# FurkanOM/tf-rpn

Hardware: AMD Instinct MI355X
Metric: proposal images/sec at 500x500x3 VOC batch; NMS boxes/sec (higher is better)
Workload: dtype f16x3; 1 GPU; configs[1]: 500x500x3 synthetic batch=8 per GPU, vgg16 backbone + RPN head, 9 anchors/cell, decode + NMS(300), 1xMI355X; per_gpu_batch=8, global_batch=8, img_size=500, anchors_per_image=8649, nms_topn=300, weights=random-init (seeded He-normal), parallelism=image-sharded dp1, one RCCL all-gather of proposals, nms_overlap=decode+NMS of step k on a second HIP stream, overlapping the convs of step k+1

## Files before the change

### tf_rpn_amd/csrc/conv_split_kernels.hip

```cpp
#include "conv_kernels.h"

#include <cmath>
#include <cstdlib>
#include <cstring>
#include <mutex>
#include <unordered_map>

#ifndef RPN_PIN
#define RPN_PIN 1
#endif
#if RPN_PIN
#define RPN_PIN_LOADS() __builtin_amdgcn_sched_barrier(0)
#else
#define RPN_PIN_LOADS() ((void)0)
#endif

#ifdef RPN_STAMP
__device__ unsigned long long g_rpn_stamps[8192 * 32];
#define RPN_STAMP_AT(k)                                                                                    \
    do {                                                                                                   \
        if (threadIdx.x == 0 && blockIdx.x < 8192 && (k) < 32)                                             \
            g_rpn_stamps[blockIdx.x * 32 + (k)] = __builtin_readcyclecounter();                            \
    } while (0)
#define RPN_STAMP_VAL(k, v)                                                                                \
    do {                                                                                                   \
        if (threadIdx.x == 0 && blockIdx.x < 8192) g_rpn_stamps[blockIdx.x * 32 + (k)] = (v);             \
    } while (0)
extern "C" int rpn_debug_read_stamps(unsigned long long *out, int n)
{
    return (int)hipMemcpyFromSymbol(out, HIP_SYMBOL(g_rpn_stamps), (size_t)n * 8);
}
#else
#define RPN_STAMP_AT(k) ((void)0)
#define RPN_STAMP_VAL(k, v) ((void)0)
#endif

namespace rpn {

__device__ __forceinline__ void wave_sync()
{
    __builtin_amdgcn_fence(__ATOMIC_RELEASE, "wavefront");
    __builtin_amdgcn_wave_barrier();
    __builtin_amdgcn_fence(__ATOMIC_ACQUIRE, "wavefront");
}

using f32x16 = __attribute__((ext_vector_type(16))) float;
using bf16x8 = __attribute__((ext_vector_type(8))) __bf16;
using f16x8 = __attribute__((ext_vector_type(8))) _Float16;
using u32x4 = __attribute__((ext_vector_type(4))) unsigned;

constexpr int TWS = 32;
constexpr int HW = TWS + 2;
constexpr int kStagePad = 4;

template <bool F16> struct Half;
template <> struct Half<false> {
    using vec = bf16x8;
    using elem = __bf16;
    static __device__ __forceinline__ f32x16 mfma(u32x4 a, u32x4 b, f32x16 c)
    {
        return __builtin_amdgcn_mfma_f32_32x32x16_bf16(__builtin_bit_cast(bf16x8, a), __builtin_bit_cast(bf16x8, b), c,
                                                       0, 0, 0);
    }
};
template <> struct Half<true> {
    using vec = f16x8;
    using elem = _Float16;
    static __device__ __forceinline__ f32x16 mfma(u32x4 a, u32x4 b, f32x16 c)
    {
        return __builtin_amdgcn_mfma_f32_32x32x16_f16(__builtin_bit_cast(f16x8, a), __builtin_bit_cast(f16x8, b), c, 0,
                                                      0, 0);
    }
};

template <bool F16>
__device__ __forceinline__ uint4 split_piece(const float (&x)[8], bool lo, unsigned *status = nullptr)
{
    using E = typename Half<F16>::elem;
    typename Half<F16>::vec v;
    if constexpr (F16) {
        if (status && !lo) {
            const float m = fmaxf(fmaxf(fmaxf(fabsf(x[0]), fabsf(x[1])), fmaxf(fabsf(x[2]), fabsf(x[3]))),
                                  fmaxf(fmaxf(fabsf(x[4]), fabsf(x[5])), fmaxf(fabsf(x[6]), fabsf(x[7]))));
            float nan_probe = 0.0f;
#pragma unroll
            for (int k = 0; k < 8; ++k) nan_probe = fmaf(x[k], 0.0f, nan_probe);
            if (!(m <= 65504.0f) || nan_probe != 0.0f) atomicOr(status, 1u );
        }
    }
#pragma unroll
    for (int k = 0; k < 8; ++k) {
        const E h = (E)x[k];
        v[k] = lo ? (E)(x[k] - (float)h) : h;
    }
    return __builtin_bit_cast(uint4, v);
}

template <bool F16>
__device__ __forceinline__ float join(unsigned short hi, unsigned short lo)
{
    using E = typename Half<F16>::elem;
    return (float)__builtin_bit_cast(E, hi) + (float)__builtin_bit_cast(E, lo);
}

using f32x4 = __attribute__((ext_vector_type(4))) float;

template <bool F16>
__device__ __forceinline__ f32x4 mfma16(u32x4 a, u32x4 b, f32x4 c)
{
    if constexpr (F16)
        return __builtin_amdgcn_mfma_f32_16x16x32_f16(__builtin_bit_cast(f16x8, a), __builtin_bit_cast(f16x8, b), c, 0, 0, 0);
    else
        return __builtin_amdgcn_mfma_f32_16x16x32_bf16(__builtin_bit_cast(bf16x8, a), __builtin_bit_cast(bf16x8, b), c, 0, 0, 0);
}

__device__ __forceinline__ int halo_swz(int hx) { return hx & 6; }

__device__ __forceinline__ int xcd_remap_s(int bid, int nwg)
{
    const int q = nwg >> 3, r = nwg & 7, xcd = bid & 7;
    return (xcd < r ? xcd * (q + 1) : r * (q + 1) + (xcd - r) * q) + (bid >> 3);
}

struct SplitConvArgs {
    const uint4 *x;
    const uint4 *w;
    const float *bias;
    void *out;
    int B, H, W, Cin, Cout, cout_pad;
    float out_scale;
    int act, out_f32;
    unsigned *sched;
    unsigned *status;
    const float *img;
    const uint4 *w1;
    const float *b1;
    float scale1;
    long long slab_floats;
    int ktree;
};

template <int TH, int WN, int BBUF, int NW, bool F16, bool POOL, bool B1 = false>
__global__ void __launch_bounds__(64 * NW, NW / 2)
conv3x3_split_kernel(SplitConvArgs a, int tiles_x, int tiles_y, int n_tiles)
{
    constexpr int NT = 64 * NW;
    constexpr int WM = NW / WN;
    constexpr int MI = TH / WM;
    constexpr int NI = 2;
    constexpr int BN = WN * NI * 32;
    constexpr int HP = (TH + 2) * HW;
    constexpr int A_PIECES = HP * 4;
    constexpr int A_ROUNDS = (A_PIECES + NT - 1) / NT;
    constexpr int A_RPS = (A_ROUNDS + 2) / 3;
    constexpr int B_PIECES = 3 * BN * 4;
    constexpr int B_ROUNDS = B_PIECES / NT;
    static_assert(MI * WM == TH && B_PIECES % NT == 0, "tile shape");
    constexpr int STAGE_LD = 64 + kStagePad;
    constexpr int ABUF = HP * 4 + 4;
    constexpr int PW = TWS + 4;
    constexpr int PATCH_F = B1 ? (TH + 4) * PW * 3 : 0;
    static_assert(!B1 || (WN == 1 && POOL && BBUF == 2), "B1: the 64 -> 64 pooled instantiations only");
    constexpr int LDS_PIPE = 2 * ABUF + BBUF * B_PIECES;
    constexpr int LDS_STAGE = (NW * 32 * STAGE_LD * 4 + 15) / 16;
    constexpr int LDS_UINT4 = (LDS_PIPE > LDS_STAGE ? LDS_PIPE : LDS_STAGE) + (PATCH_F + 3) / 4;

    __shared__ uint4 lds[LDS_UINT4];
    u32x4 *As = reinterpret_cast<u32x4 *>(lds);
    u32x4 *Bs = reinterpret_cast<u32x4 *>(lds) + 2 * ABUF;

    const int tid = threadIdx.x;
    const int lane = tid & 63;
    const int wave = tid >> 6;
    const int wm = wave / WN, wn = wave % WN;
    const int lm = lane & 31, kh = lane >> 5;

    int nt, mt;
    {
        const int m_tiles = tiles_x * tiles_y * a.B;
        const int XN = n_tiles >= 8 ? 8 : (n_tiles >= 4 ? 4 : (n_tiles >= 2 ? 2 : 1)), XM = 8 / XN;
        const int NTl = (n_tiles + XN - 1) / XN;
        const int xcd = blockIdx.x & 7, slot = blockIdx.x >> 3;
        nt = (slot % NTl) * XN + (xcd % XN);
        mt = (slot / NTl) * XM + (xcd / XN);
        if (nt >= n_tiles || mt >= m_tiles) return;
    }
    const int tx = mt % tiles_x;
    mt /= tiles_x;
    const int ty = mt % tiles_y;
    const int img = mt / tiles_y;
    const int oy0 = ty * TH, ox0 = tx * TWS, n0 = nt * BN;

    const int chunks = a.Cin >> 4;
    const int steps = chunks * 3;
    const size_t in_pix_stride = (size_t)chunks * 4;
    const uint4 *__restrict__ xin = B1 ? nullptr : a.x + (size_t)img * a.H * a.W * in_pix_stride;

    constexpr int A_SLOTS = 3 * A_RPS;
    constexpr unsigned kOob = 0x80000000u;
    const __amdgpu_buffer_rsrc_t xrsrc = __builtin_amdgcn_make_buffer_rsrc(
        const_cast<uint4 *>(xin), (short)0, (int)((size_t)a.H * a.W * in_pix_stride * 16), 0x00020000);
    unsigned a_goff[A_SLOTS];
    int a_loff[A_SLOTS];
#pragma unroll
    for (int R = 0; R < (B1 ? 0 : A_SLOTS); ++R) {
        const int e = R * NT + tid;
        const int pix = e >> 2, pc = e & 3;
        const int hy = pix / HW, hx = pix - hy * HW;
        const int iy = oy0 - 1 + hy, ix = ox0 - 1 + hx;
        const bool piece = e < A_PIECES;
        const bool inimg = piece && iy >= 0 && iy < a.H && ix >= 0 && ix < a.W;
        a_loff[R] = piece ? (pix * 4 + (pc ^ ((hx >> 2) & 3))) : HP * 4;
        a_goff[R] = inimg ? (unsigned)((((size_t)iy * a.W + ix) * in_pix_stride + pc) * 16) : kOob;
    }
    u32x4 b_reg[B_ROUNDS];
    u32x4 a_reg[A_RPS];
#define RPN_LOAD_B(STEP)                                                                               \
    {                                                                                                  \
        const u32x4 *src_ = reinterpret_cast<const u32x4 *>(a.w) + ((size_t)(STEP) * 3 * a.cout_pad + n0) * 4;   \
        _Pragma("unroll") for (int i_ = 0; i_ < B_ROUNDS; ++i_) {                                      \
            const int e_ = tid + i_ * NT;                                                              \
            const int t_ = e_ / (BN * 4), rem_ = e_ - t_ * (BN * 4);                \
            b_reg[i_] = src_[(size_t)t_ * a.cout_pad * 4 + rem_];                                      \
        }                                                                                              \
    }
#define RPN_STORE_B(BUF)                                                                               \
    {                                                                                                  \
        _Pragma("unroll") for (int i_ = 0; i_ < B_ROUNDS; ++i_) {                                      \
            const int e_ = tid + i_ * NT;                                                              \
            const int t_ = e_ / (BN * 4), rem_ = e_ - t_ * (BN * 4);                                   \
            const int n_ = rem_ >> 2, pc_ = rem_ & 3;                                                  \
            Bs[(((BUF) * 3 + t_) * BN + n_) * 4 + (pc_ ^ ((n_ >> 2) & 3))] = b_reg[i_];                \
        }                                                                                              \
    }
#define RPN_LOAD_A(CHUNK, R) \
    __builtin_bit_cast(u32x4, __builtin_amdgcn_raw_buffer_load_b128(xrsrc, a_goff[R], (CHUNK) * 64, 0))

    constexpr int NBLK = (HP + 15) / 16;
    constexpr int QB = B1 ? (NBLK + NW - 1) / NW : 1;
    constexpr int QPS = (QB + 2) / 3;
    float *patchf = reinterpret_cast<float *>(lds + (LDS_PIPE > LDS_STAGE ? LDS_PIPE : LDS_STAGE));
    const int lr = lane & 15, kg = lane >> 4;
    u32x4 phi[QB], plo[QB];
    int pdst[QB];
    float b1_max = 0.0f;
    unsigned pin = 0;
    u32x4 w1hi = {0, 0, 0, 0}, w1lo = {0, 0, 0, 0};
    f32x4 b1v = {0.f, 0.f, 0.f, 0.f};
    (void)patchf; (void)lr; (void)kg; (void)pin; (void)phi; (void)plo; (void)pdst; (void)w1hi; (void)w1lo; (void)b1v;
    (void)b1_max;
#define RPN_B1_LOADW(CHUNK)                                                                            \
    {                                                                                                  \
        const u32x4 *w1_ = reinterpret_cast<const u32x4 *>(a.w1) + ((CHUNK) * 16 + lr) * 8 + kg;       \
        w1hi = w1_[0];                                                                                 \
        w1lo = w1_[4];                                                                                 \
        b1v = *reinterpret_cast<const f32x4 *>(a.b1 + (CHUNK) * 16 + 4 * kg);                          \
    }
#define RPN_B1_BLOCK(Q, BUF)                                                                           \
    {                                                                                                  \
        f32x4 c_ = {0.f, 0.f, 0.f, 0.f};                                                               \
        c_ = mfma16<F16>(w1lo, phi[Q], c_);                                                            \
        c_ = mfma16<F16>(w1hi, plo[Q], c_);                                                            \
        c_ = mfma16<F16>(w1hi, phi[Q], c_);                                                            \
        using E_ = typename Half<F16>::elem;                                                           \
        using h4_ = __attribute__((ext_vector_type(4))) E_;                                            \
        const bool in_ = (pin >> (Q)) & 1u;                                                            \
        h4_ hv_, lv_;                                                                                  \
        _Pragma("unroll") for (int r_ = 0; r_ < 4; ++r_) {                                             \
            float v_ = fmaxf(c_[r_] * a.scale1 + b1v[r_], 0.0f);                                       \
            v_ = in_ ? v_ : 0.0f;                                                                      \
            b1_max = fmaxf(b1_max, v_);                                                                \
            const E_ h_ = (E_)v_;                                                                      \
            hv_[r_] = h_;                                                                              \
            lv_[r_] = (E_)(v_ - (float)h_);                                                            \
        }                                                                                              \
        char *d_ = reinterpret_cast<char *>(As + (BUF) * ABUF);                                        \
        *reinterpret_cast<uint2 *>(d_ + pdst[Q]) = __builtin_bit_cast(uint2, hv_);                     \
        *reinterpret_cast<uint2 *>(d_ + (pdst[Q] ^ 16)) = __builtin_bit_cast(uint2, lv_);              \
    }
    if constexpr (B1) {
        const float *ximg = a.img + (size_t)img * a.H * a.W * 3;
        for (int e = tid; e < PATCH_F; e += NT) {
            const int pr = e / (PW * 3), rem = e - pr * (PW * 3);
            const int iy = oy0 - 2 + pr, ix = ox0 - 2 + rem / 3;
            patchf[e] = (iy >= 0 && iy < a.H && ix >= 0 && ix < a.W) ? ximg[((size_t)iy * a.W + ix) * 3 + rem % 3] : 0.0f;
        }
    }

    f32x16 acc[MI][NI];
#pragma unroll
    for (int i = 0; i < MI; ++i)
#pragma unroll
        for (int j = 0; j < NI; ++j)
#pragma unroll
            for (int e = 0; e < 16; ++e) acc[i][j][e] = 0.0f;

    int a_off[3];
#pragma unroll
    for (int s3 = 0; s3 < 3; ++s3) a_off[s3] = (lm + s3) * 4 + ((2 * kh) ^ (((lm + s3) >> 2) & 3));
    int b_off[NI];
#pragma unroll
    for (int j = 0; j < NI; ++j) {
        const int n = wn * (NI * 32) + j * 32 + lm;
        b_off[j] = n * 4 + ((2 * kh) ^ ((n >> 2) & 3));
    }

    if constexpr (B1) {
        RPN_LOAD_B(0);
        RPN_B1_LOADW(0);
        RPN_STORE_B(0);
        __syncthreads();
        int koff[8];
#pragma unroll
        for (int j = 0; j < 8; ++j) {
            const int k = 8 * kg + j;
            koff[j] = k < 27 ? (k / 9) * (PW * 3) + (k % 9) : -1;
        }
#pragma unroll
        for (int q = 0; q < QB; ++q) {
            const int p = (wave + NW * q) * 16 + lr;
            const bool valid = p < HP;
            const int pp = valid ? p : HP - 1;
            const int hy = pp / HW, hx = pp - hy * HW;
            const int base = (hy * PW + hx) * 3;
            float xs[8];
#pragma unroll
            for (int j = 0; j < 8; ++j) xs[j] = koff[j] >= 0 ? patchf[base + koff[j]] : 0.0f;
            phi[q] = __builtin_bit_cast(u32x4, split_piece<F16>(xs, false));
            plo[q] = __builtin_bit_cast(u32x4, split_piece<F16>(xs, true));
            const int iy = oy0 - 1 + hy, ix = ox0 - 1 + hx;
            if (iy >= 0 && iy < a.H && ix >= 0 && ix < a.W) pin |= 1u << q;
            pdst[q] = valid ? (pp * 4 + ((2 * (kg >> 1)) ^ ((hx >> 2) & 3))) * 16 + (kg & 1) * 8 : HP * 4 * 16 + (kg & 1) * 8;
        }
#pragma unroll
        for (int q = 0; q < QB; ++q) RPN_B1_BLOCK(q, 0);
    } else {
#pragma unroll
        for (int R = 0; R < A_SLOTS; ++R) As[a_loff[R]] = RPN_LOAD_A(0, R);
        RPN_LOAD_B(0);
        RPN_STORE_B(0);
    }
    __syncthreads();

    int abuf = 0, bbuf = 0;
#pragma unroll 1
    for (int chunk = 0; chunk < chunks; ++chunk) {
        const int next_chunk = chunk + 1 < chunks ? chunk + 1 : chunk;
#pragma unroll
        for (int row = 0; row < 3; ++row) {
            const int step = chunk * 3 + row;
            RPN_LOAD_B(step + 1 < steps ? step + 1 : step);
            if constexpr (B1) {
                if (row == 0) RPN_B1_LOADW(next_chunk);
            } else {
#pragma unroll
                for (int q = 0; q < A_RPS; ++q) a_reg[q] = RPN_LOAD_A(next_chunk, row * A_RPS + q);
            }
            if constexpr (NW == 4) RPN_PIN_LOADS();

            const u32x4 *arow = As + (abuf * ABUF + (wm * MI + row) * HW * 4);
#pragma unroll
            for (int s = 0; s < 3; ++s) {
                u32x4 ahi[MI], alo[MI], bhi[NI], blo[NI];
#pragma unroll
                for (int i = 0; i < MI; ++i) {
                    ahi[i] = arow[i * HW * 4 + a_off[s]];
                    alo[i] = arow[i * HW * 4 + (a_off[s] ^ 1)];
                }
#pragma unroll
                for (int j = 0; j < NI; ++j) {
                    bhi[j] = Bs[(bbuf * 3 + s) * BN * 4 + b_off[j]];
                    blo[j] = Bs[(bbuf * 3 + s) * BN * 4 + (b_off[j] ^ 1)];
                }
#pragma unroll
                for (int i = 0; i < MI; ++i)
#pragma unroll
                    for (int j = 0; j < NI; ++j) {
                        acc[i][j] = Half<F16>::mfma(alo[i], bhi[j], acc[i][j]);
                        acc[i][j] = Half<F16>::mfma(ahi[i], blo[j], acc[i][j]);
                        acc[i][j] = Half<F16>::mfma(ahi[i], bhi[j], acc[i][j]);
                    }
            }

            if (BBUF == 1) __syncthreads();
            RPN_STORE_B(BBUF == 2 ? (bbuf ^ 1) : 0);
            if constexpr (B1) {
#pragma unroll
                for (int q = row * QPS; q < (row + 1) * QPS && q < QB; ++q) RPN_B1_BLOCK(q, abuf ^ 1);
            } else {
#pragma unroll
                for (int q = 0; q < A_RPS; ++q) As[(abuf ^ 1) * ABUF + a_loff[row * A_RPS + q]] = a_reg[q];
            }
            __syncthreads();
            if (BBUF == 2) bbuf ^= 1;
        }
        abuf ^= 1;
    }

#undef RPN_LOAD_B
#undef RPN_STORE_B
#undef RPN_LOAD_A
#undef RPN_B1_LOADW
#undef RPN_B1_BLOCK
    if constexpr (B1 && F16) {
        if (a.status && !(b1_max <= 65504.0f)) atomicOr(a.status, 1u );
    }
    float *stage = reinterpret_cast<float *>(lds) + wave * (32 * STAGE_LD);
    float bias_v[NI];
#pragma unroll
    for (int j = 0; j < NI; ++j) {
        const int n = n0 + wn * (NI * 32) + j * 32 + lm;
        bias_v[j] = (a.bias && n < a.Cout) ? a.bias[n] : 0.0f;
    }
    const float act_lo = a.act == ACT_LINEAR ? -INFINITY : 0.0f;
    const float act_hi = a.act == ACT_RELU6 ? 6.0f : INFINITY;
    const int cout_chunks = a.Cout >> 4;
    const int nbase = n0 + wn * (NI * 32);
    const int pix_bytes = a.out_f32 ? a.Cout * 4 : cout_chunks * 64;
    auto store_stage = [&](int npx_log2, int oy, int oxb, int OHo, int OWo) {
        if (oy >= OHo) return;
        const long long row_off = (((long long)img * OHo + oy) * OWo + oxb) * (long long)pix_bytes;
        const __amdgpu_buffer_rsrc_t ors = __builtin_amdgcn_make_buffer_rsrc(reinterpret_cast<char *>(a.out) + row_off, (short)0,
                                                                              (OWo - oxb) * pix_bytes, 0x00020000);
        if (a.out_f32) {
            const int rounds = (16 << npx_log2) >> 6;
            const int px_l = lane >> 4, q_l = lane & 15;
            const int n = nbase + 4 * q_l;
            unsigned voff = n < a.Cout ? (unsigned)(px_l * pix_bytes + n * 4) : 0x80000000u;
#pragma unroll
            for (int rd = 0; rd < rounds; ++rd) {
                const u32x4 v = *reinterpret_cast<const u32x4 *>(&stage[(rd * 4 + px_l) * STAGE_LD + 4 * q_l]);
                __builtin_amdgcn_raw_buffer_store_b128(v, ors, voff, 0, 0);
                voff += (unsigned)(4 * pix_bytes);
            }
        } else {
            const int rounds2 = (8 << npx_log2) >> 6;
            const int px2 = lane >> 3, q2 = lane & 7;
            const int cl = q2 >> 1, hf = q2 & 1;
            const int n = nbase + cl * 16;
            unsigned voff = n < a.Cout ? (unsigned)(px2 * pix_bytes + (n >> 4) * 64 + hf * 32) : 0x80000000u;
#pragma unroll
            for (int rd = 0; rd < rounds2; ++rd) {
                float xs[8];
                const float *src = &stage[(rd * 8 + px2) * STAGE_LD + cl * 16 + hf * 8];
                const float4 v0 = *reinterpret_cast<const float4 *>(src);
                const float4 v1 = *reinterpret_cast<const float4 *>(src + 4);
                xs[0] = v0.x; xs[1] = v0.y; xs[2] = v0.z; xs[3] = v0.w;
                xs[4] = v1.x; xs[5] = v1.y; xs[6] = v1.z; xs[7] = v1.w;
                const u32x4 hi = __builtin_bit_cast(u32x4, split_piece<F16>(xs, false, a.status));
                const u32x4 lo = __builtin_bit_cast(u32x4, split_piece<F16>(xs, true, nullptr));
                __builtin_amdgcn_raw_buffer_store_b128(hi, ors, voff, 0, 0);
                __builtin_amdgcn_raw_buffer_store_b128(lo, ors, voff + 16u, 0, 0);
                voff += (unsigned)(8 * pix_bytes);
            }
        }
    };

    if constexpr (POOL) {
        static_assert(!POOL || (MI % 2 == 0), "pooling needs an even number of rows per wave");
        const int OHo = a.H >> 1, OWo = a.W >> 1;
#pragma unroll
        for (int ip = 0; ip < MI / 2; ++ip) {
#pragma unroll
            for (int j = 0; j < NI; ++j)
#pragma unroll
                for (int e2 = 0; e2 < 8; ++e2) {
                    const float v0 = fmaxf(acc[2 * ip][j][2 * e2], acc[2 * ip][j][2 * e2 + 1]);
                    const float v1 = fmaxf(acc[2 * ip + 1][j][2 * e2], acc[2 * ip + 1][j][2 * e2 + 1]);
                    const int m2 = (e2 & 1) + 4 * (e2 >> 1) + 2 * kh;
                    stage[m2 * STAGE_LD + j * 32 + lm] = fminf(fmaxf(fmaxf(v0, v1) * a.out_scale + bias_v[j], act_lo), act_hi);
                }
            wave_sync();
            store_stage(4, (oy0 + wm * MI + 2 * ip) >> 1, ox0 >> 1, OHo, OWo);
            wave_sync();
        }
    } else {
#pragma unroll
        for (int i = 0; i < MI; ++i) {
#pragma unroll
            for (int j = 0; j < NI; ++j)
#pragma unroll
                for (int e = 0; e < 16; ++e) {
                    const int m = (e & 3) + 8 * (e >> 2) + 4 * kh;
                    stage[m * STAGE_LD + j * 32 + lm] = fminf(fmaxf(acc[i][j][e] * a.out_scale + bias_v[j], act_lo), act_hi);
                }
            wave_sync();
            store_stage(5, oy0 + wm * MI + i, ox0, a.H, a.W);
            wave_sync();
        }
    }
}


#ifdef RPN_NOSTORE
#define RPN_STORE_INDEX(i) ((i) & 63)
#else
#define RPN_STORE_INDEX(i) (i)
#endif

template <bool F16, bool POOL, int RW, int NW, int NJ = 4>
__device__ __forceinline__ void split16_epilogue(f32x4 (&acc)[RW * 2][NJ], float *lds_f, const SplitConvArgs &a, int img,
                                                 int oy0, int ox0, int n0, int wave, int wm, int wn, int lane,
                                                 int stamp_base = -1 )
{
    (void)stamp_base;
    asm volatile("" : "+v"(lane));
    constexpr int MT = RW * 2;
    constexpr int CW = 16 * NJ;
    constexpr int STAGE_LD = CW + kStagePad;
    constexpr int PP = CW / 4;
    const int lr = lane & 15, kg = lane >> 4;
    float *stage = lds_f + wave * (32 * STAGE_LD);
    float bias_v[NJ];
#pragma unroll
    for (int j = 0; j < NJ; ++j) {
        const int n = n0 + wn * CW + j * 16 + lr;
        bias_v[j] = (a.bias && n < a.Cout) ? a.bias[n] : 0.0f;
    }
    const float act_lo = a.act == ACT_LINEAR ? -INFINITY : 0.0f;
    const float act_hi = a.act == ACT_RELU6 ? 6.0f : INFINITY;
    const int cout_chunks = a.Cout >> 4;
    const int nbase = n0 + wn * CW;
    const int pix_bytes = a.out_f32 ? a.Cout * 4 : cout_chunks * 64;
    constexpr int PXR = 64 / PP;
    const int px_l = lane / PP, q_l = lane % PP;
    auto store_stage = [&](int npx_log2, int oy, int oxb, int OHo, int OWo) {
        if (oy >= OHo) return;
        const int rounds = (PP << npx_log2) >> 6;
        const long long row_off = (((long long)img * OHo + oy) * OWo + oxb) * (long long)pix_bytes;
        const __amdgpu_buffer_rsrc_t ors = __builtin_amdgcn_make_buffer_rsrc(reinterpret_cast<char *>(a.out) + row_off, (short)0,
                                                                              (OWo - oxb) * pix_bytes, 0x00020000);
        if (a.out_f32) {
            const int n = nbase + 4 * q_l;
            unsigned voff = n < a.Cout ? (unsigned)(px_l * pix_bytes + n * 4) : 0x80000000u;
#pragma unroll
            for (int rd = 0; rd < rounds; ++rd) {
                const u32x4 v = *reinterpret_cast<const u32x4 *>(&stage[(rd * PXR + px_l) * STAGE_LD + 4 * q_l]);
#ifdef RPN_NOSTORE
                __builtin_amdgcn_raw_buffer_store_b128(v, ors, (unsigned)(lane * 16), 0, 0);
#else
                __builtin_amdgcn_raw_buffer_store_b128(v, ors, voff, 0, 0);
#endif
                voff += (unsigned)(PXR * pix_bytes);
            }
        } else {
            constexpr int LPP = CW / 8;
            constexpr int PXR2 = 64 / LPP;
            const int px2 = lane / LPP, q2 = lane % LPP;
            const int cl = q2 >> 1, hf = q2 & 1;
            const int n = nbase + cl * 16;
            unsigned voff = n < a.Cout ? (unsigned)(px2 * pix_bytes + (n >> 4) * 64 + hf * 32) : 0x80000000u;
            const int rounds2 = (1 << npx_log2) / PXR2;
#pragma unroll
            for (int rd = 0; rd < rounds2; ++rd) {
                float xs[8];
                const float *src = &stage[(rd * PXR2 + px2) * STAGE_LD + cl * 16 + hf * 8];
                const float4 v0 = *reinterpret_cast<const float4 *>(src);
                const float4 v1 = *reinterpret_cast<const float4 *>(src + 4);
                xs[0] = v0.x; xs[1] = v0.y; xs[2] = v0.z; xs[3] = v0.w;
                xs[4] = v1.x; xs[5] = v1.y; xs[6] = v1.z; xs[7] = v1.w;
                const u32x4 hi = __builtin_bit_cast(u32x4, split_piece<F16>(xs, false, a.status));
                const u32x4 lo = __builtin_bit_cast(u32x4, split_piece<F16>(xs, true, nullptr));
#ifdef RPN_NOSTORE
                __builtin_amdgcn_raw_buffer_store_b128(hi, ors, (unsigned)(lane * 32), 0, 0);
                __builtin_amdgcn_raw_buffer_store_b128(lo, ors, (unsigned)(lane * 32 + 16), 0, 0);
#else
                __builtin_amdgcn_raw_buffer_store_b128(hi, ors, voff, 0, 0);
                __builtin_amdgcn_raw_buffer_store_b128(lo, ors, voff + 16u, 0, 0);
#endif
                voff += (unsigned)(PXR2 * pix_bytes);
            }
        }
    };

    if constexpr (POOL) {
        const int OHo = a.H >> 1, OWo = a.W >> 1;
#pragma unroll
        for (int hf = 0; hf < 2; ++hf)
#pragma unroll
            for (int j = 0; j < NJ; ++j)
#pragma unroll
                for (int r2 = 0; r2 < 2; ++r2) {
                    const float v0 = fmaxf(acc[hf][j][2 * r2], acc[hf][j][2 * r2 + 1]);
                    const float v1 = fmaxf(acc[(MT - 2) + hf][j][2 * r2], acc[(MT - 2) + hf][j][2 * r2 + 1]);
                    const int px2 = 8 * hf + 2 * kg + r2;
                    stage[px2 * STAGE_LD + j * 16 + lr] = fminf(fmaxf(fmaxf(v0, v1) * a.out_scale + bias_v[j], act_lo), act_hi);
                }
        wave_sync();
        store_stage(4, (oy0 + 2 * wm) >> 1, ox0 >> 1, OHo, OWo);
    } else {
#pragma unroll
        for (int i = 0; i < RW; ++i) {
#pragma unroll
            for (int hf = 0; hf < 2; ++hf)
#pragma unroll
                for (int j = 0; j < NJ; ++j)
#pragma unroll
                    for (int r = 0; r < 4; ++r) {
                        const int px = 16 * hf + 4 * kg + r;
                        stage[px * STAGE_LD + j * 16 + lr] =
                            fminf(fmaxf(acc[i * 2 + hf][j][r] * a.out_scale + bias_v[j], act_lo), act_hi);
                    }
            wave_sync();
            if (stamp_base >= 0) RPN_STAMP_AT(stamp_base + 2 * i);
            store_stage(5, oy0 + RW * wm + i, ox0, a.H, a.W);
            wave_sync();
            if (stamp_base >= 0) RPN_STAMP_AT(stamp_base + 2 * i + 1);
        }
    }
}

template <int TH, int WN, int NW, bool F16, bool POOL>
__global__ void __launch_bounds__(64 * NW, NW == 8 ? 2 : 2)
conv3x3_split16_kernel(SplitConvArgs a, int tiles_x, int tiles_y, int n_tiles)
{
    constexpr int NT = 64 * NW, BN = 64 * WN;
    constexpr int WM = NW / WN, RW = TH / WM;
    constexpr int MT = RW * 2;
    constexpr int HP = (TH + 2) * HW;
    constexpr int PPP = 8;
    constexpr int ABUF = HP * PPP + 8;
    constexpr int A_PIECES = HP * PPP;
    constexpr int A_ROUNDS = (A_PIECES + NT - 1) / NT;
    constexpr int A_RPS = (A_ROUNDS + 2) / 3, A_SLOTS = 3 * A_RPS;
    constexpr int B_PIECES = 3 * BN * PPP;
    constexpr int B_ROUNDS = B_PIECES / NT;
    constexpr int STAGE_LD = 64 + kStagePad;
    constexpr int LDS_PIPE = 2 * ABUF + B_PIECES;
    constexpr int LDS_STAGE = (NW * 32 * STAGE_LD * 4 + 15) / 16;
    constexpr int LDS_UINT4 = LDS_PIPE > LDS_STAGE ? LDS_PIPE : LDS_STAGE;
    static_assert(RW * WM == TH && RW >= 1 && B_PIECES % NT == 0 && (!POOL || RW == 2), "tile shape");

    __shared__ uint4 lds[LDS_UINT4];
    u32x4 *As = reinterpret_cast<u32x4 *>(lds);
    u32x4 *Bs = reinterpret_cast<u32x4 *>(lds) + 2 * ABUF;

    const int tid = threadIdx.x;
    const int lane = tid & 63;
    const int wave = tid >> 6;
    const int wm = wave / WN, wn = wave % WN;
    const int lr = lane & 15, kg = lane >> 4;

    int nt, mt;
    {
        const int m_tiles = tiles_x * tiles_y * a.B;
        const int XN = n_tiles >= 8 ? 8 : (n_tiles >= 4 ? 4 : (n_tiles >= 2 ? 2 : 1)), XM = 8 / XN;
        const int NTl = (n_tiles + XN - 1) / XN;
        const int xcd = blockIdx.x & 7, slot = blockIdx.x >> 3;
        nt = (slot % NTl) * XN + (xcd % XN);
        mt = (slot / NTl) * XM + (xcd / XN);
        if (nt >= n_tiles || mt >= m_tiles) return;
    }
    const int tx = mt % tiles_x;
    mt /= tiles_x;
    const int ty = mt % tiles_y;
    const int img = mt / tiles_y;
    const int oy0 = ty * TH, ox0 = tx * TWS, n0 = nt * BN;
    RPN_STAMP_AT(0);
    RPN_STAMP_VAL(1, ((unsigned long long)__builtin_amdgcn_s_getreg((31 << 11) | 20) << 32) |
                         (unsigned)__builtin_amdgcn_s_getreg((31 << 11) | 4));

    const int all_chunks = a.Cin >> 5;
    int c_begin = (int)((long long)blockIdx.y * all_chunks / gridDim.y);
    int chunks = (int)((long long)(blockIdx.y + 1) * all_chunks / gridDim.y);
    int c_fold = -1;
    constexpr bool KT = TH == 4 && NW == 4 && !POOL;
    if (KT && a.ktree) {
        const int per = 4 / (int)gridDim.y, l0 = (int)blockIdx.y * per;
        c_begin = ktree_cut(all_chunks, l0);
        chunks = ktree_cut(all_chunks, l0 + per);
        if (per == 2) c_fold = ktree_cut(all_chunks, l0 + 1);
    }
    const int steps = chunks * 3;
    const size_t in_pix_stride = (size_t)(a.Cin >> 4) * 4;
    const uint4 *__restrict__ xin = a.x + (size_t)img * a.H * a.W * in_pix_stride;

    constexpr unsigned kOob = 0x80000000u;
    const __amdgpu_buffer_rsrc_t xrsrc = __builtin_amdgcn_make_buffer_rsrc(
        const_cast<uint4 *>(xin), (short)0, (int)((size_t)a.H * a.W * in_pix_stride * 16), 0x00020000);
    unsigned a_goff[A_SLOTS];
    int a_loff[A_SLOTS];
#pragma unroll
    for (int R = 0; R < A_SLOTS; ++R) {
        const int e = R * NT + tid;
        const int pix = e >> 3, q = e & 7;
        const int hy = pix / HW, hx = pix - hy * HW;
        const int iy = oy0 - 1 + hy, ix = ox0 - 1 + hx;
        const bool piece = e < A_PIECES;
        const bool inimg = piece && iy >= 0 && iy < a.H && ix >= 0 && ix < a.W;
        const int kgq = (q >> 2) * 2 + ((q >> 1) & 1), lo = q & 1;
        a_loff[R] = piece ? (pix * PPP + ((lo * 4 + kgq) ^ halo_swz(hx))) : HP * PPP;
        a_goff[R] = inimg ? (unsigned)((((size_t)iy * a.W + ix) * in_pix_stride + q) * 16) : kOob;
    }
    u32x4 b_reg[B_ROUNDS];
    u32x4 a_reg[A_RPS];
#define RPN16_LOAD_B(STEP)                                                                                   \
    {                                                                                                        \
        const u32x4 *src_ = reinterpret_cast<const u32x4 *>(a.w) + ((size_t)(STEP) * 3 * a.cout_pad + n0) * PPP; \
        _Pragma("unroll") for (int i_ = 0; i_ < B_ROUNDS; ++i_) {                                            \
            const int e_ = tid + i_ * NT;                                                                    \
            const int t_ = e_ / (BN * PPP), rem_ = e_ - t_ * (BN * PPP);                                     \
            b_reg[i_] = src_[(size_t)t_ * a.cout_pad * PPP + rem_];                                          \
        }                                                                                                    \
    }
#define RPN16_STORE_B()                                                                                      \
    {                                                                                                        \
        _Pragma("unroll") for (int i_ = 0; i_ < B_ROUNDS; ++i_) {                                            \
            const int e_ = tid + i_ * NT;                                                                    \
            const int t_ = e_ / (BN * PPP), rem_ = e_ - t_ * (BN * PPP);                                     \
            Bs[t_ * BN * PPP + rem_] = b_reg[i_];        \
        }                                                                                                    \
    }
#define RPN16_LOAD_A(CHUNK, R) \
    __builtin_bit_cast(u32x4, __builtin_amdgcn_raw_buffer_load_b128(xrsrc, a_goff[R], (CHUNK) * 128, 0))

    f32x4 acc[MT][4];
    f32x4 leaf0[KT ? MT : 1][KT ? 4 : 1];
    (void)leaf0;
#pragma unroll
    for (int m = 0; m < MT; ++m)
#pragma unroll
        for (int j = 0; j < 4; ++j) {
            acc[m][j] = f32x4{0.f, 0.f, 0.f, 0.f};
            if constexpr (KT) leaf0[m][j] = f32x4{0.f, 0.f, 0.f, 0.f};
        }

    int a_off[3][2];
#pragma unroll
    for (int s3 = 0; s3 < 3; ++s3)
#pragma unroll
        for (int hf = 0; hf < 2; ++hf) {
            const int hx = 16 * hf + lr + s3;
            a_off[s3][hf] = hx * PPP + (kg ^ halo_swz(hx));
        }
    int b_off[4];
#pragma unroll
    for (int j = 0; j < 4; ++j) {
        const int n = wn * 64 + j * 16 + lr;
        b_off[j] = n * PPP + (kg ^ ((n >> 1) & 7));
    }

#pragma unroll
    for (int R = 0; R < A_SLOTS; ++R) As[a_loff[R]] = RPN16_LOAD_A(c_begin, R);
    RPN16_LOAD_B(3 * c_begin);
    RPN16_STORE_B();
    __syncthreads();
    RPN_STAMP_AT(2);

    int abuf = 0;
#pragma unroll 1
    for (int chunk = c_begin; chunk < chunks; ++chunk) {
        const int next_chunk = chunk + 1 < chunks ? chunk + 1 : chunk;
#pragma unroll
        for (int row = 0; row < 3; ++row) {
            const int step = chunk * 3 + row;
            RPN16_LOAD_B(step + 1 < steps ? step + 1 : step);
#pragma unroll
            for (int q = 0; q < A_RPS; ++q) a_reg[q] = RPN16_LOAD_A(next_chunk, row * A_RPS + q);
            RPN_PIN_LOADS();

            const u32x4 *arow = As + (abuf * ABUF + (RW * wm + row) * HW * PPP);
#pragma unroll
            for (int s = 0; s < 3; ++s) {
                u32x4 ahi[MT], alo[MT], bhi[4], blo[4];
#pragma unroll
                for (int m = 0; m < MT; ++m) {
                    const int idx = (m >> 1) * HW * PPP + a_off[s][m & 1];
                    ahi[m] = arow[idx];
                    alo[m] = arow[idx ^ 4];
                }
#pragma unroll
                for (int j = 0; j < 4; ++j) {
                    bhi[j] = Bs[s * BN * PPP + b_off[j]];
                    blo[j] = Bs[s * BN * PPP + (b_off[j] ^ 4)];
                }
#pragma unroll
                for (int m = 0; m < MT; ++m)
#pragma unroll
                    for (int j = 0; j < 4; ++j) {
                        acc[m][j] = mfma16<F16>(alo[m], bhi[j], acc[m][j]);
                        acc[m][j] = mfma16<F16>(ahi[m], blo[j], acc[m][j]);
                        acc[m][j] = mfma16<F16>(ahi[m], bhi[j], acc[m][j]);
                    }
            }
            __syncthreads();
            RPN16_STORE_B();
#pragma unroll
            for (int q = 0; q < A_RPS; ++q) As[(abuf ^ 1) * ABUF + a_loff[row * A_RPS + q]] = a_reg[q];
            __syncthreads();
        }
        abuf ^= 1;
        RPN_STAMP_AT(4 + chunk);
        if constexpr (KT) {
            if (chunk + 1 == c_fold) {
#pragma unroll
                for (int m = 0; m < MT; ++m)
#pragma unroll
                    for (int j = 0; j < 4; ++j) {
                        leaf0[m][j] = acc[m][j];
                        acc[m][j] = f32x4{0.f, 0.f, 0.f, 0.f};
                    }
            }
        }
    }
    if constexpr (KT) {
        if (c_fold >= 0) {
#pragma unroll
            for (int m = 0; m < MT; ++m)
#pragma unroll
                for (int j = 0; j < 4; ++j) acc[m][j] = leaf0[m][j] + acc[m][j];
        }
    }
#undef RPN16_LOAD_B
#undef RPN16_STORE_B
#undef RPN16_LOAD_A

    if (gridDim.y > 1) {
        SplitConvArgs ar = a;
        ar.bias = nullptr;
        ar.act = ACT_LINEAR;
        ar.out_f32 = 1;
        ar.out = reinterpret_cast<float *>(a.out) + (size_t)blockIdx.y * a.slab_floats;
        split16_epilogue<F16, POOL, RW, NW>(acc, reinterpret_cast<float *>(lds), ar, img, oy0, ox0, n0, wave, wm, wn, lane);
    } else {
        split16_epilogue<F16, POOL, RW, NW>(acc, reinterpret_cast<float *>(lds), a, img, oy0, ox0, n0, wave, wm, wn, lane);
    }
    RPN_STAMP_AT(3);
}

#ifndef RPN_DMA_SCHED
#define RPN_DMA_SCHED 1
#endif
#define RPN_LDS_PTR(p) ((__attribute__((address_space(3))) void *)(p))

struct TileWalk {
    int n_tiles, m_tiles, tiles_x, tiles_y, XN, XM, NTl, n_slots, xcd, slot_stride, bn;
    __device__ __forceinline__ bool decode(int slot, int &img, int &oy0, int &ox0, int &n0) const
    {
        const int nt = (slot % NTl) * XN + (xcd % XN);
        int mt = (slot / NTl) * XM + (xcd / XN);
        if (nt >= n_tiles || mt >= m_tiles) return false;
        const int tx = mt % tiles_x;
        mt /= tiles_x;
        const int ty = mt % tiles_y;
        img = mt / tiles_y;
        oy0 = ty * 8; ox0 = tx * TWS; n0 = nt * bn;
        return true;
    }
    __device__ __forceinline__ int next(int slot, int &img, int &oy0, int &ox0, int &n0) const
    {
        for (; slot < n_slots; slot += slot_stride)
            if (decode(slot, img, oy0, ox0, n0)) return slot;
        return -1;
    }
    __device__ __forceinline__ int settle(int ticket, unsigned *queue) const
    {
        int img, oy0, ox0, n0, slot = ticket + slot_stride;
        while (slot < n_slots && !decode(slot, img, oy0, ox0, n0)) slot = (int)atomicAdd(queue, 1u) + slot_stride;
        return slot;
    }
};

template <int NW, int A_INSTR, int A_PIECES>
__device__ __forceinline__ unsigned halo_source_offset(int j, int wave, int lane, int im, int y0, int x0, int H, int W,
                                                       int in_pix_stride)
{
    int ln = lane;
    asm volatile("" : "+v"(ln));
    int k = j * NW + wave;
    if (k >= A_INSTR) k -= A_INSTR;
    const int e = k * 64 + ln;
    const int pix = e >> 3, ps = e & 7;
    const int hy = pix / HW, hx = pix - hy * HW;
    const int iy = y0 - 1 + hy, ix = x0 - 1 + hx;
    const bool in = e < A_PIECES && iy >= 0 && iy < H && ix >= 0 && ix < W;
    const int lg = ps ^ halo_swz(hx);
    const int q = (((lg & 3) >> 1) << 2) | ((lg & 1) << 1) | (lg >> 2);
    return in ? (unsigned)((((im * H + iy) * W + ix) * in_pix_stride + q) * 16) : 0x80000000u;
}

template <bool F16, bool POOL, int BN, bool KTREE = false>
__global__ void __launch_bounds__(512, 2)
conv3x3_split16_dma_kernel(SplitConvArgs a, int tiles_x, int tiles_y, int n_tiles)
{
    static_assert(!KTREE || (BN == 64 && !POOL), "K tree: the 64-wide tile has the registers for two more accumulator sets");
    constexpr int TH = 8, NW = 8, WN = 2, RW = 2, MT = 4, PPP = 8;
    constexpr int NJ = BN / (16 * WN);
    constexpr int B_PER_WAVE = BN * PPP / 64 / NW;
    constexpr int HP = (TH + 2) * HW;
    constexpr int A_INSTR = (HP * PPP + 63) / 64;
    constexpr int ABUF = A_INSTR * 64;
    constexpr int A_PER_WAVE = (A_INSTR + NW - 1) / NW;
    constexpr int BSLOT = BN * PPP;
    constexpr int B_AT = ABUF, DUMP = B_AT + 3 * BSLOT, A1_AT = DUMP + 64;
    constexpr int STAGE_PIECES = NW * 32 * (16 * NJ + kStagePad) * 4 / 16;
    constexpr int LDS_UINT4 = A1_AT + (ABUF > STAGE_PIECES ? ABUF : STAGE_PIECES);
    static_assert(A_PER_WAVE <= 9 && RW * (NW / WN) == TH && MT == 2 * RW && LDS_UINT4 * 16 <= 160 * 1024 &&
                      (BN == 128 || BN == 64), "tile shape");

    __shared__ uint4 lds[LDS_UINT4];
    u32x4 *As = reinterpret_cast<u32x4 *>(lds);
    u32x4 *Bs = reinterpret_cast<u32x4 *>(lds) + B_AT;

    const int tid = threadIdx.x;
    const int lane = tid & 63;
    const int wave = __builtin_amdgcn_readfirstlane(tid >> 6);
    const int wm = wave / WN, wn = wave % WN;
    const int lr = lane & 15, kg = lane >> 4;

    const int m_tiles = tiles_x * tiles_y * a.B;
    const int XN = n_tiles >= 8 ? 8 : (n_tiles >= 4 ? 4 : (n_tiles >= 2 ? 2 : 1)), XM = 8 / XN;
    const int NTl = (n_tiles + XN - 1) / XN, MTl = (m_tiles + XM - 1) / XM;
    const int xcd = blockIdx.x & 7;
    const int slot_stride = gridDim.x >> 3;
    const TileWalk walk{n_tiles, m_tiles, tiles_x, tiles_y, XN, XM, NTl, NTl * MTl, xcd, slot_stride, BN};
#define next_tile(SLOT, IMG, OY0, OX0, N0) walk.next((SLOT), (IMG), (OY0), (OX0), (N0))

    const int all_chunks = a.Cin >> 5;
    int cb = 0, chunks = all_chunks;
    if constexpr (KTREE) {
        if (gridDim.y == 2) {
            const int mid = ktree_cut(all_chunks, 2);
            cb = blockIdx.y ? mid : 0;
            chunks = blockIdx.y ? all_chunks - mid : mid;
            a.out = reinterpret_cast<float *>(a.out) + (size_t)blockIdx.y * a.slab_floats;
        }
    }
    const int total_taps = chunks * 9, tap0 = cb * 9;
    const int in_pix_stride = (a.Cin >> 4) * 4;
    const __amdgpu_buffer_rsrc_t xrsrc = __builtin_amdgcn_make_buffer_rsrc(
        const_cast<uint4 *>(a.x), (short)0, (int)((size_t)a.B * a.H * a.W * in_pix_stride * 16), 0x00020000);
    const __amdgpu_buffer_rsrc_t wrsrc = __builtin_amdgcn_make_buffer_rsrc(
        const_cast<uint4 *>(a.w), (short)0, (int)((size_t)all_chunks * 9 * a.cout_pad * 128), 0x00020000);
    const int w_tap_bytes = a.cout_pad * 128;

#define halo_goff(J, IM, Y0, X0) halo_source_offset<NW, A_INSTR, HP * PPP>((J), wave, lane, (IM), (Y0), (X0), a.H, a.W, in_pix_stride)
    const unsigned b_voff = (unsigned)(((B_PER_WAVE * wave) * 64 + lane) * 16);

#define RPN_DMA_A(J, GOFF, SOFF, BUF)                                                                             \
    {                                                                                                             \
        const int k0_ = (J) * NW + wave, k_ = k0_ < A_INSTR ? k0_ : k0_ - A_INSTR;            \
        u32x4 *dst_ = As + (BUF) * A1_AT + k_ * 64;                                                               \
        __builtin_amdgcn_raw_ptr_buffer_load_lds(xrsrc, RPN_LDS_PTR(dst_), 16, (GOFF), (SOFF), 0, 0);             \
    }
#define RPN_DMA_B(SOFF, SLOT)                                                                                     \
    {                                                                                                             \
        u32x4 *dst_ = Bs + (SLOT) * BSLOT + (B_PER_WAVE * wave) * 64;                                             \
        __builtin_amdgcn_raw_ptr_buffer_load_lds(wrsrc, RPN_LDS_PTR(dst_), 16, b_voff, (SOFF), 0, 0);             \
                                        \
        if constexpr (B_PER_WAVE == 2)                                                                            \
            __builtin_amdgcn_raw_ptr_buffer_load_lds(wrsrc, RPN_LDS_PTR(dst_), 16, b_voff, (SOFF), 1024, 0);      \
    }

    int a_off[3][2];
#pragma unroll
    for (int s3 = 0; s3 < 3; ++s3)
#pragma unroll
        for (int hf = 0; hf < 2; ++hf) {
            const int hx = 16 * hf + lr + s3;
            a_off[s3][hf] = hx * PPP + (kg ^ halo_swz(hx));
        }
    int b_off[NJ];
#pragma unroll
    for (int j = 0; j < NJ; ++j) {
        const int n = wn * (16 * NJ) + j * 16 + lr;
        b_off[j] = n * PPP + (kg ^ ((n >> 1) & 7));
    }

    const bool dyn = a.sched != nullptr;
    int *tile_q = reinterpret_cast<int *>(lds + DUMP);
    int img = 0, oy0 = 0, ox0 = 0, n0 = 0;
    int cur;
    if (dyn) {
        cur = blockIdx.x >> 3;
        if (!walk.decode(cur, img, oy0, ox0, n0)) {
            if (tid == 0) tile_q[0] = walk.settle((int)atomicAdd(a.sched + xcd, 1u), a.sched + xcd);
            __syncthreads();
            cur = __builtin_amdgcn_readfirstlane(tile_q[0]);
            __syncthreads();
            if (cur >= walk.n_slots || !walk.decode(cur, img, oy0, ox0, n0)) cur = -1;
        }
    } else {
        cur = next_tile(blockIdx.x >> 3, img, oy0, ox0, n0);
    }
#define RPN_SCHED_EXIT()                                                                                          \
    if (dyn && tid == 0) {                                                                                        \
        __threadfence();                                                                                          \
        if (atomicAdd(a.sched + 8 + xcd, 1u) == (gridDim.x >> 3) - 1 && atomicAdd(a.sched + 16, 1u) == 7) {       \
            _Pragma("unroll") for (int i_ = 0; i_ < 17; ++i_) a.sched[i_] = 0u;                                   \
        }                                                                                                         \
    }
    if (cur < 0) {
        RPN_SCHED_EXIT();
        return;
    }
    RPN_STAMP_AT(0);
    RPN_STAMP_VAL(1, ((unsigned long long)__builtin_amdgcn_s_getreg((31 << 11) | 20) << 32) |
                         (unsigned)__builtin_amdgcn_s_getreg((31 << 11) | 4));

    u32x4 fx0[4], fx1[4], fw[2][2 * NJ];
#define RPN_X_ADDR(BUF, ROW, S, I, II)                          \
    (As[(BUF) * A1_AT + (RW * wm + (ROW) + (I)) * HW * PPP + (a_off[S][(II) >> 1] ^ (((II) & 1) ? 4 : 0))])
#define RPN_W_ADDR(S, II)                                                           \
    (Bs[(S) * BSLOT + (b_off[(II) >> 1] ^ (((II) & 1) ? 4 : 0))])

    unsigned a_goff[A_PER_WAVE];
#pragma unroll
    for (int j = 0; j < A_PER_WAVE; ++j) a_goff[j] = halo_goff(j, img, oy0, ox0);
#pragma unroll
    for (int j = 0; j < A_PER_WAVE; ++j) RPN_DMA_A(j, a_goff[j], cb * 128, 0);
#pragma unroll
    for (int t = 0; t < 3; ++t) RPN_DMA_B((tap0 + t) * w_tap_bytes + n0 * (PPP * 16), t);
    asm volatile("s_waitcnt vmcnt(0)" ::: "memory");
    __builtin_amdgcn_s_barrier();
#pragma unroll
    for (int i = 0; i < 2 * NJ; ++i) fw[0][i] = RPN_W_ADDR(0, i);
#pragma unroll
    for (int i = 0; i < 4; ++i) fx0[i] = RPN_X_ADDR(0, 0, 0, 0, i);
    asm volatile("s_waitcnt lgkmcnt(0)" ::: "memory");
    __builtin_amdgcn_s_barrier();

    int gt = 3;
    int tile_no = 0;
    for (;;) {
        int nimg = 0, noy0 = 0, nox0 = 0, nn0 = 0;
        int nxt = -1;
        unsigned ticket = 0;
        if (dyn) {
            if (tid == 0) ticket = atomicAdd(a.sched + xcd, 1u);
        } else {
            nxt = next_tile(cur + slot_stride, nimg, noy0, nox0, nn0);
        }
        f32x4 acc[MT][NJ];
        f32x4 t01[KTREE ? MT : 1][KTREE ? NJ : 1], t23[KTREE ? MT : 1][KTREE ? NJ : 1];
        (void)t01; (void)t23;
#pragma unroll
        for (int m = 0; m < MT; ++m)
#pragma unroll
            for (int j = 0; j < NJ; ++j) acc[m][j] = f32x4{0.f, 0.f, 0.f, 0.f};

#pragma unroll 1
        for (int pair = 0; pair < (chunks >> 1); ++pair) {
#pragma unroll
            for (int T = 0; T < 18; ++T) {
                const int c2 = T / 9, s9 = T % 9;
                const int CS = T & 1, CB = c2 & 1, CR = s9 / 3, CC = s9 % 3;
                const int NS = (T + 1) & 1, NB = ((T + 1) / 9) & 1, NR = ((T + 1) % 9) / 3, NC = ((T + 1) % 9) % 3;
                {
                    int tap = gt, nb = n0;
                    if (gt >= total_taps) {
                        if (nxt >= 0) { tap = gt - total_taps; nb = nn0; }
                        else tap = total_taps - 1;
                    }
#ifndef RPN_EXP_NO_DMA
                    RPN_DMA_B((tap0 + tap) * w_tap_bytes + nb * (PPP * 16), s9 % 3);
#endif
                    ++gt;
                }
                if (dyn && pair == 0) {
                    if (T == 4 && tid == 0) tile_q[tile_no & 1] = walk.settle((int)ticket, a.sched + xcd);
                    if (T == 6) {
                        const int sl = __builtin_amdgcn_readfirstlane(tile_q[tile_no & 1]);
                        nxt = (sl < walk.n_slots && walk.decode(sl, nimg, noy0, nox0, nn0)) ? sl : -1;
                    }
                }
                if (T == 9 && nxt >= 0 && pair == (chunks >> 1) - 1) {
#pragma unroll
                    for (int j = 0; j < A_PER_WAVE; ++j) a_goff[j] = halo_goff(j, nimg, noy0, nox0);
                }
                if (s9 < A_PER_WAVE) {
                    const int nc = 2 * pair + c2 + 1;
#ifndef RPN_EXP_NO_DMA
                    RPN_DMA_A(s9, a_goff[s9], (cb + (nc < chunks ? nc : (nxt >= 0 ? 0 : chunks - 1))) * 128, (c2 + 1) & 1);
#endif
                }
#pragma unroll
                for (int i = 0; i < 2 * NJ; ++i) {
#ifndef RPN_EXP_NO_LDSREAD
                    if (i < 4) fx1[i] = RPN_X_ADDR(CB, CR, CC, 1, i);
#endif
                    acc[i / NJ][i % NJ] = mfma16<F16>(fx0[2 * (i / NJ) + 1], fw[CS][2 * (i % NJ)], acc[i / NJ][i % NJ]);
                }
#pragma unroll
                for (int i = 0; i < 2 * NJ; ++i) {
                    acc[i / NJ][i % NJ] = mfma16<F16>(fx0[2 * (i / NJ)], fw[CS][2 * (i % NJ) + 1], acc[i / NJ][i % NJ]);
                    acc[i / NJ][i % NJ] = mfma16<F16>(fx0[2 * (i / NJ)], fw[CS][2 * (i % NJ)], acc[i / NJ][i % NJ]);
                }
#if RPN_DMA_SCHED
                if (s9 < A_PER_WAVE) __builtin_amdgcn_sched_group_barrier(0x020, B_PER_WAVE + 1, 0);
                else __builtin_amdgcn_sched_group_barrier(0x020, B_PER_WAVE, 0);
#pragma unroll
                for (int i = 0; i < 4; ++i) {
                    __builtin_amdgcn_sched_group_barrier(0x100, 1, 0);
                    __builtin_amdgcn_sched_group_barrier(0x008, 1, 0);
                }
                __builtin_amdgcn_sched_group_barrier(0x008, 6 * NJ - 4, 0);
                __builtin_amdgcn_sched_barrier(0);
#endif
#pragma unroll
                for (int i = 0; i < 2 * NJ; ++i) {
#ifndef RPN_EXP_NO_LDSREAD
                    fw[NS][i] = RPN_W_ADDR(NC, i);
#else
                    fw[NS][i] = fw[CS][i];
#endif
                    acc[2 + i / NJ][i % NJ] = mfma16<F16>(fx1[2 * (i / NJ) + 1], fw[CS][2 * (i % NJ)], acc[2 + i / NJ][i % NJ]);
                }
#pragma unroll
                for (int i = 0; i < 2 * NJ; ++i) {
#ifndef RPN_EXP_NO_LDSREAD
                    if (i < 4) fx0[i] = RPN_X_ADDR(NB, NR, NC, 0, i);
#endif
                    acc[2 + i / NJ][i % NJ] = mfma16<F16>(fx1[2 * (i / NJ)], fw[CS][2 * (i % NJ) + 1], acc[2 + i / NJ][i % NJ]);
                    acc[2 + i / NJ][i % NJ] = mfma16<F16>(fx1[2 * (i / NJ)], fw[CS][2 * (i % NJ)], acc[2 + i / NJ][i % NJ]);
                }
#if RPN_DMA_SCHED
#pragma unroll
                for (int i = 0; i < 2 * NJ; ++i) {
                    __builtin_amdgcn_sched_group_barrier(0x100, 1, 0);
                    __builtin_amdgcn_sched_group_barrier(0x008, 1, 0);
                }
#pragma unroll
                for (int i = 0; i < 4; ++i) {
                    __builtin_amdgcn_sched_group_barrier(0x100, 1, 0);
                    __builtin_amdgcn_sched_group_barrier(0x008, 2, 0);
                }
                if constexpr (4 * NJ - 8 > 0) __builtin_amdgcn_sched_group_barrier(0x008, 4 * NJ - 8, 0);
                __builtin_amdgcn_sched_barrier(0);
#endif
#ifdef RPN_EXP_HALF_BARRIERS
                if ((T & 1) == 0) continue;
#endif
                if (T == 0 && pair == 0) {
                } else if constexpr (B_PER_WAVE == 2) {
                    if (s9 < A_PER_WAVE) asm volatile("s_waitcnt vmcnt(3)" ::: "memory");
                    else asm volatile("s_waitcnt vmcnt(2)" ::: "memory");
                } else {
                    if (s9 < A_PER_WAVE) asm volatile("s_waitcnt vmcnt(2)" ::: "memory");
                    else asm volatile("s_waitcnt vmcnt(1)" ::: "memory");
                }
                asm volatile("s_waitcnt lgkmcnt(0)" ::: "memory");
                __builtin_amdgcn_s_barrier();
#if RPN_DMA_SCHED
                __builtin_amdgcn_sched_barrier(0);
#endif
                if (s9 == 8 && tile_no == 1) RPN_STAMP_AT(4 + 2 * pair + c2);
                if constexpr (KTREE) {
                    if (s9 == 8) {
                        const int done = cb + 2 * pair + c2 + 1;
                        const bool e0 = done == ktree_cut(all_chunks, 1), e1 = done == ktree_cut(all_chunks, 2),
                                   e2 = done == ktree_cut(all_chunks, 3);
                        if (e0 || e1 || e2) {
#pragma unroll
                            for (int m = 0; m < MT; ++m)
#pragma unroll
                                for (int j = 0; j < NJ; ++j) {
                                    if (e0) t01[m][j] = acc[m][j];
                                    else if (e1) t01[m][j] = t01[m][j] + acc[m][j];
                                    else t23[m][j] = acc[m][j];
                                    acc[m][j] = f32x4{0.f, 0.f, 0.f, 0.f};
                                }
                        }
                    }
                }
            }
        }
        if constexpr (KTREE) {
#pragma unroll
            for (int m = 0; m < MT; ++m)
#pragma unroll
                for (int j = 0; j < NJ; ++j) {
                    if (gridDim.y == 2) acc[m][j] = blockIdx.y == 0 ? t01[m][j] : t23[m][j] + acc[m][j];
                    else acc[m][j] = t01[m][j] + (t23[m][j] + acc[m][j]);
                }
        }
        if (tile_no < 2) RPN_STAMP_AT(20 + 6 * tile_no);
        asm volatile("s_waitcnt vmcnt(0)" ::: "memory");
        if (tile_no < 2) RPN_STAMP_AT(21 + 6 * tile_no);
#ifdef RPN_EXP_NO_EPILOGUE
#pragma unroll
        for (int m = 0; m < MT; ++m)
#pragma unroll
            for (int j = 0; j < NJ; ++j) asm volatile("" ::"v"(acc[m][j]));
#elif defined(RPN_STAMP)
        split16_epilogue<F16, POOL, RW, NW, NJ>(acc, reinterpret_cast<float *>(lds + A1_AT), a, img, oy0, ox0, n0, wave, wm, wn, lane,
                                                tile_no < 2 ? 22 + 6 * tile_no : -1);
#else
        split16_epilogue<F16, POOL, RW, NW, NJ>(acc, reinterpret_cast<float *>(lds + A1_AT), a, img, oy0, ox0, n0, wave, wm, wn, lane);
#endif
        if (tile_no == 1) RPN_STAMP_AT(3);
        if (nxt < 0) break;
        __builtin_amdgcn_s_barrier();
        if (tile_no == 0) RPN_STAMP_AT(2);
        cur = nxt; img = nimg; oy0 = noy0; ox0 = nox0; n0 = nn0;
        gt -= total_taps;
        ++tile_no;
    }
#undef RPN_X_ADDR
#undef RPN_W_ADDR
#undef next_tile
#undef halo_goff
    asm volatile("s_waitcnt vmcnt(0)" ::: "memory");
    RPN_SCHED_EXIT();
#undef RPN_SCHED_EXIT
#undef RPN_DMA_A
#undef RPN_DMA_B
}

#ifdef RPN_LAB
template <bool F16, bool POOL>
__global__ void __launch_bounds__(256) __attribute__((amdgpu_waves_per_eu(1, 1)))
conv3x3_split16_dma4_kernel(SplitConvArgs a, int tiles_x, int tiles_y, int n_tiles)
{
    constexpr int BN = 128, TH = 8, NW = 4, RW = 4, MT = 8, NJ = 4, PPP = 8;
    constexpr int B_PER_WAVE = BN * PPP / 64 / NW;
    constexpr int HP = (TH + 2) * HW;
    constexpr int A_INSTR = (HP * PPP + 63) / 64;
    constexpr int ABUF = A_INSTR * 64;
    constexpr int A_PER_WAVE = 11;
    constexpr int BSLOT = BN * PPP;
    constexpr int B_AT = ABUF, DUMP = B_AT + 3 * BSLOT, A1_AT = DUMP + 64;
    constexpr int STAGE_AT = A1_AT + ABUF;
    constexpr int STAGE_LD = 16 * NJ + kStagePad;
    constexpr int STAGE_PIECES = NW * 16 * STAGE_LD * 4 / 16;
    constexpr int LDS_UINT4 = STAGE_AT + STAGE_PIECES;
    static_assert((A_INSTR + NW - 1) / NW == A_PER_WAVE && LDS_UINT4 * 16 <= 160 * 1024, "tile shape");

    __shared__ uint4 lds[LDS_UINT4];
    u32x4 *As = reinterpret_cast<u32x4 *>(lds);
    u32x4 *Bs = reinterpret_cast<u32x4 *>(lds) + B_AT;

    const int tid = threadIdx.x;
    const int lane = tid & 63;
    const int wave = __builtin_amdgcn_readfirstlane(tid >> 6);
    const int wm = wave >> 1, wn = wave & 1;
    const int lr = lane & 15, kg = lane >> 4;

    const int m_tiles = tiles_x * tiles_y * a.B;
    const int XN = n_tiles >= 8 ? 8 : (n_tiles >= 4 ? 4 : (n_tiles >= 2 ? 2 : 1)), XM = 8 / XN;
    const int NTl = (n_tiles + XN - 1) / XN, MTl = (m_tiles + XM - 1) / XM;
    const int xcd = blockIdx.x & 7;
    const int slot_stride = gridDim.x >> 3;
    const TileWalk walk{n_tiles, m_tiles, tiles_x, tiles_y, XN, XM, NTl, NTl * MTl, xcd, slot_stride, BN};

    const int chunks = a.Cin >> 5;
    const int total_taps = chunks * 9;
    const int in_pix_stride = (a.Cin >> 4) * 4;
    const __amdgpu_buffer_rsrc_t xrsrc = __builtin_amdgcn_make_buffer_rsrc(
        const_cast<uint4 *>(a.x), (short)0, (int)((size_t)a.B * a.H * a.W * in_pix_stride * 16), 0x00020000);
    const __amdgpu_buffer_rsrc_t wrsrc = __builtin_amdgcn_make_buffer_rsrc(
        const_cast<uint4 *>(a.w), (short)0, (int)((size_t)total_taps * a.cout_pad * 128), 0x00020000);
    const int w_tap_bytes = a.cout_pad * 128;

#define halo_goff4(J, IM, Y0, X0) halo_source_offset<NW, A_INSTR, HP * PPP>((J), wave, lane, (IM), (Y0), (X0), a.H, a.W, in_pix_stride)
    const unsigned b_voff = (unsigned)(((B_PER_WAVE * wave) * 64 + lane) * 16);
#define RPN4_DMA_A(J, GOFF, SOFF, BUF)                                                                            \
    {                                                                                                             \
        const int k0_ = (J) * NW + wave, k_ = k0_ < A_INSTR ? k0_ : k0_ - A_INSTR;                                \
        u32x4 *dst_ = As + (BUF) * A1_AT + k_ * 64;                                                               \
        __builtin_amdgcn_raw_ptr_buffer_load_lds(xrsrc, RPN_LDS_PTR(dst_), 16, (GOFF), (SOFF), 0, 0);             \
    }
#define RPN4_DMA_B(SOFF, SLOT)                                                                                    \
    {                                                                                                             \
        u32x4 *dst_ = Bs + (SLOT) * BSLOT + (B_PER_WAVE * wave) * 64;                                             \
        __builtin_amdgcn_raw_ptr_buffer_load_lds(wrsrc, RPN_LDS_PTR(dst_), 16, b_voff, (SOFF), 0, 0);             \
        __builtin_amdgcn_raw_ptr_buffer_load_lds(wrsrc, RPN_LDS_PTR(dst_), 16, b_voff, (SOFF), 1024, 0);          \
        __builtin_amdgcn_raw_ptr_buffer_load_lds(wrsrc, RPN_LDS_PTR(dst_), 16, b_voff, (SOFF), 2048, 0);          \
        __builtin_amdgcn_raw_ptr_buffer_load_lds(wrsrc, RPN_LDS_PTR(dst_), 16, b_voff, (SOFF), 3072, 0);          \
    }

    int a_off[3][2];
#pragma unroll
    for (int s3 = 0; s3 < 3; ++s3)
#pragma unroll
        for (int hf = 0; hf < 2; ++hf) {
            const int hx = 16 * hf + lr + s3;
            a_off[s3][hf] = hx * PPP + (kg ^ halo_swz(hx));
        }
    int b_off[NJ];
#pragma unroll
    for (int j = 0; j < NJ; ++j) {
        const int n = wn * (16 * NJ) + j * 16 + lr;
        b_off[j] = n * PPP + (kg ^ ((n >> 1) & 7));
    }

    int img = 0, oy0 = 0, ox0 = 0, n0 = 0;
    int cur = walk.next(blockIdx.x >> 3, img, oy0, ox0, n0);
    if (cur < 0) return;

    u32x4 fxA[4], fxB[4], fw[2][2 * NJ];
#define RPN4_X_ADDR(BUF, ROW, S, I, II)                                                                          \
    (As[(BUF) * A1_AT + (RW * wm + (ROW) + (I)) * HW * PPP + (a_off[S][(II) >> 1] ^ (((II) & 1) ? 4 : 0))])
#define RPN4_W_ADDR(S, II) (Bs[(S) * BSLOT + (b_off[(II) >> 1] ^ (((II) & 1) ? 4 : 0))])

    unsigned a_goff[A_PER_WAVE];
#pragma unroll
    for (int j = 0; j < A_PER_WAVE; ++j) a_goff[j] = halo_goff4(j, img, oy0, ox0);
#pragma unroll
    for (int j = 0; j < A_PER_WAVE; ++j) RPN4_DMA_A(j, a_goff[j], 0, 0);
#pragma unroll
    for (int t = 0; t < 3; ++t) RPN4_DMA_B(t * w_tap_bytes + n0 * (PPP * 16), t);
    asm volatile("s_waitcnt vmcnt(0)" ::: "memory");
    __builtin_amdgcn_s_barrier();
#pragma unroll
    for (int i = 0; i < 2 * NJ; ++i) fw[0][i] = RPN4_W_ADDR(0, i);
#pragma unroll
    for (int i = 0; i < 4; ++i) fxA[i] = RPN4_X_ADDR(0, 0, 0, 0, i);
    asm volatile("s_waitcnt lgkmcnt(0)" ::: "memory");
    __builtin_amdgcn_s_barrier();

    f32x4 done[MT][NJ];
    float d_bias[NJ];
    int d_img = 0, d_oy0 = 0, d_ox0 = 0, d_n0 = 0;
    bool pending = false;
#pragma unroll
    for (int m = 0; m < MT; ++m)
#pragma unroll
        for (int j = 0; j < NJ; ++j) done[m][j] = f32x4{0.f, 0.f, 0.f, 0.f};
#pragma unroll
    for (int j = 0; j < NJ; ++j) d_bias[j] = 0.0f;
    float *stage = reinterpret_cast<float *>(lds + STAGE_AT) + wave * (16 * STAGE_LD);
    const long long out_bytes = (long long)a.B * (POOL ? a.H >> 1 : a.H) * (POOL ? a.W >> 1 : a.W) * a.Cout * 4;
    const __amdgpu_buffer_rsrc_t orsrc = __builtin_amdgcn_make_buffer_rsrc(a.out, (short)0, (int)out_bytes, 0x00020000);
    const float act_lo = a.act == ACT_LINEAR ? -INFINITY : 0.0f;
    const float act_hi = a.act == ACT_RELU6 ? 6.0f : INFINITY;
    const int cout_chunks = a.Cout >> 4;
    constexpr int PP = 16 * NJ / 4;

#define RPN4_EPI_STAGE(STEP)                                                                                       \
    {                                                                                                              \
        if constexpr (POOL) {                                                                                      \
            const int st_ = (STEP) & 3, rp_ = st_ >> 1, h_ = st_ & 1;                                                            \
            _Pragma("unroll") for (int j = 0; j < NJ; ++j)                                                         \
                _Pragma("unroll") for (int r2 = 0; r2 < 2; ++r2) {                                                 \
                    const float v0 = fmaxf(done[(2 * rp_) * 2 + h_][j][2 * r2], done[(2 * rp_) * 2 + h_][j][2 * r2 + 1]);            \
                    const float v1 = fmaxf(done[(2 * rp_ + 1) * 2 + h_][j][2 * r2], done[(2 * rp_ + 1) * 2 + h_][j][2 * r2 + 1]);    \
                    stage[(2 * kg + r2) * STAGE_LD + j * 16 + lr] =                                                \
                        fminf(fmaxf(fmaxf(v0, v1) * a.out_scale + d_bias[j], act_lo), act_hi);                     \
                }                                                                                                  \
        } else {                                                                                                   \
            const int st_ = (STEP) & 7, r_ = st_ >> 1, h_ = st_ & 1;                                                       \
            _Pragma("unroll") for (int j = 0; j < NJ; ++j)                                                         \
                _Pragma("unroll") for (int e = 0; e < 4; ++e)                                                      \
                    stage[(4 * kg + e) * STAGE_LD + j * 16 + lr] =                                                 \
                        fminf(fmaxf(done[r_ * 2 + h_][j][e] * a.out_scale + d_bias[j], act_lo), act_hi);           \
        }                                                                                                          \
        wave_sync();                                                                                               \
    }
#define RPN4_EPI_STORE(STEP)                                                                                       \
    {                                                                                                              \
        constexpr int NPX_ = POOL ? 8 : 16;                                                                        \
        const int st_ = (STEP) & (POOL ? 3 : 7), h_ = st_ & 1;                                                     \
        const int OHo_ = POOL ? a.H >> 1 : a.H, OWo_ = POOL ? a.W >> 1 : a.W;                                      \
        const int oy_ = POOL ? (d_oy0 + RW * wm + 2 * (st_ >> 1)) >> 1 : d_oy0 + RW * wm + (st_ >> 1);             \
        const int oxb_ = POOL ? (d_ox0 >> 1) + 8 * h_ : d_ox0 + 16 * h_;                                           \
        const int nbase_ = d_n0 + wn * (16 * NJ);                                                                  \
        const int row_ = (d_img * OHo_ + oy_) * OWo_;                                                              \
        int ln_ = lane;                                                                                            \
        asm volatile("" : "+v"(ln_));                                                                              \
        _Pragma("unroll") for (int rd = 0; rd < NPX_ * PP / 64; ++rd) {                                            \
            const int e = rd * 64 + ln_;                                                                           \
            const int px = e / PP, q = e % PP;                                                                     \
            const int ox = oxb_ + px;                                                                              \
            if (a.out_f32) {                                                                                       \
                const int n = nbase_ + 4 * q;                                                                      \
                const bool ok = oy_ < OHo_ && ox < OWo_ && n < a.Cout;                                             \
                const u32x4 v = *reinterpret_cast<const u32x4 *>(&stage[px * STAGE_LD + 4 * q]);                   \
                __builtin_amdgcn_raw_buffer_store_b128(v, orsrc, ok ? ((row_ + ox) * a.Cout + n) * 4 : (int)0x80000000, 0, 0);   \
            } else {                                                                                               \
                const int cl = q >> 2, pc = q & 3;                                                                 \
                const int n = nbase_ + cl * 16;                                                                    \
                const bool ok = oy_ < OHo_ && ox < OWo_ && n < a.Cout;                                             \
                float xs[8];                                                                                       \
                const float *src = &stage[px * STAGE_LD + cl * 16 + (pc >> 1) * 8];                                \
                const float4 v0 = *reinterpret_cast<const float4 *>(src);                                          \
                const float4 v1 = *reinterpret_cast<const float4 *>(src + 4);                                      \
                xs[0] = v0.x; xs[1] = v0.y; xs[2] = v0.z; xs[3] = v0.w;                                            \
                xs[4] = v1.x; xs[5] = v1.y; xs[6] = v1.z; xs[7] = v1.w;                                            \
                const uint4 pv = split_piece<F16>(xs, (pc & 1) != 0, ok ? a.status : nullptr);                     \
                __builtin_amdgcn_raw_buffer_store_b128(u32x4{pv.x, pv.y, pv.z, pv.w}, orsrc,                       \
                    ok ? (((row_ + ox) * cout_chunks + (n >> 4)) * 4 + pc) * 16 : (int)0x80000000, 0, 0);          \
            }                                                                                                      \
        }                                                                                                          \
        wave_sync();                                                                                               \
    }
    constexpr int EPI_STEPS = POOL ? 4 : 8;

#define RPN4_ROW_MFMA(Q, F)                                                                                        \
    {                                                                                                              \
        _Pragma("unroll") for (int i = 0; i < 2 * NJ; ++i)                                                         \
            acc[2 * (Q) + i / NJ][i % NJ] = mfma16<F16>(F[2 * (i / NJ) + 1], fw[CS][2 * (i % NJ)], acc[2 * (Q) + i / NJ][i % NJ]);   \
        _Pragma("unroll") for (int i = 0; i < 2 * NJ; ++i) {                                                       \
            acc[2 * (Q) + i / NJ][i % NJ] = mfma16<F16>(F[2 * (i / NJ)], fw[CS][2 * (i % NJ) + 1], acc[2 * (Q) + i / NJ][i % NJ]);   \
            acc[2 * (Q) + i / NJ][i % NJ] = mfma16<F16>(F[2 * (i / NJ)], fw[CS][2 * (i % NJ)], acc[2 * (Q) + i / NJ][i % NJ]);       \
        }                                                                                                          \
    }

    int gt = 3;
    for (;;) {
        int nimg = 0, noy0 = 0, nox0 = 0, nn0 = 0;
        const int nxt = walk.next(cur + slot_stride, nimg, noy0, nox0, nn0);
        f32x4 acc[MT][NJ];
#pragma unroll
        for (int m = 0; m < MT; ++m)
#pragma unroll
            for (int j = 0; j < NJ; ++j) acc[m][j] = f32x4{0.f, 0.f, 0.f, 0.f};

#pragma unroll 1
        for (int pair = 0; pair < (chunks >> 1); ++pair) {
#ifdef RPN_EXP_W4_SYNC_EPI
            const bool epi = false;
#else
            const bool epi = pending && pair == 0;
#endif
#pragma unroll
            for (int T = 0; T < 18; ++T) {
                const int c2 = T / 9, s9 = T % 9;
                const int CS = T & 1, CB = c2 & 1, CR = s9 / 3, CC = s9 % 3;
                const int NS = (T + 1) & 1, NB = ((T + 1) / 9) & 1, NR = ((T + 1) % 9) / 3, NC = ((T + 1) % 9) % 3;
                const int nA = s9 < 5 ? 2 : (s9 == 5 ? 1 : 0);
                if (T == 9 && nxt >= 0 && pair == (chunks >> 1) - 1) {
#pragma unroll
                    for (int j = 0; j < A_PER_WAVE; ++j) a_goff[j] = halo_goff4(j, nimg, noy0, nox0);
                }
                if (T >= 1 && T <= EPI_STEPS && epi) RPN4_EPI_STAGE(T - 1);
#pragma unroll
                for (int i = 0; i < 4; ++i) fxB[i] = RPN4_X_ADDR(CB, CR, CC, 1, i);
                RPN4_ROW_MFMA(0, fxA);
                __builtin_amdgcn_sched_barrier(0);
                if (T >= 1 && T <= EPI_STEPS && epi) RPN4_EPI_STORE(T - 1);
#pragma unroll
                for (int i = 0; i < 4; ++i) fxA[i] = RPN4_X_ADDR(CB, CR, CC, 2, i);
                RPN4_ROW_MFMA(1, fxB);
                __builtin_amdgcn_sched_barrier(0);
                {
                    int tap = gt, nb = n0;
                    if (gt >= total_taps) {
                        if (nxt >= 0) { tap = gt - total_taps; nb = nn0; }
                        else tap = total_taps - 1;
                    }
                    RPN4_DMA_B(tap * w_tap_bytes + nb * (PPP * 16), s9 % 3);
                    ++gt;
                }
                if (nA > 0) {
                    const int nc = 2 * pair + c2 + 1;
                    const int soff = nc < chunks ? nc * 128 : (nxt >= 0 ? 0 : (chunks - 1) * 128);
                    if (s9 < 5) {
                        RPN4_DMA_A(2 * s9, a_goff[2 * s9], soff, (c2 + 1) & 1);
                        RPN4_DMA_A(2 * s9 + 1, a_goff[2 * s9 + 1], soff, (c2 + 1) & 1);
                    } else {
                        RPN4_DMA_A(10, a_goff[10], soff, (c2 + 1) & 1);
                    }
                }
                __builtin_amdgcn_sched_barrier(0);
#pragma unroll
                for (int i = 0; i < 4; ++i) fxB[i] = RPN4_X_ADDR(CB, CR, CC, 3, i);
                RPN4_ROW_MFMA(2, fxA);
                __builtin_amdgcn_sched_barrier(0);
#pragma unroll
                for (int i = 0; i < 2 * NJ; ++i) fw[NS][i] = RPN4_W_ADDR(NC, i);
#pragma unroll
                for (int i = 0; i < 4; ++i) fxA[i] = RPN4_X_ADDR(NB, NR, NC, 0, i);
                RPN4_ROW_MFMA(3, fxB);
                __builtin_amdgcn_sched_barrier(0);
                if (nA == 2) asm volatile("s_waitcnt vmcnt(6)" ::: "memory");
                else if (nA == 1) asm volatile("s_waitcnt vmcnt(5)" ::: "memory");
                else asm volatile("s_waitcnt vmcnt(4)" ::: "memory");
                asm volatile("s_waitcnt lgkmcnt(0)" ::: "memory");
                __builtin_amdgcn_s_barrier();
                __builtin_amdgcn_sched_barrier(0);
            }
        }
#pragma unroll
        for (int m = 0; m < MT; ++m)
#pragma unroll
            for (int j = 0; j < NJ; ++j) done[m][j] = acc[m][j];
#pragma unroll
        for (int j = 0; j < NJ; ++j) {
            const int n = n0 + wn * (16 * NJ) + j * 16 + lr;
            d_bias[j] = (a.bias && n < a.Cout) ? a.bias[n] : 0.0f;
        }
        d_img = img; d_oy0 = oy0; d_ox0 = ox0; d_n0 = n0;
        pending = true;
#ifdef RPN_EXP_W4_SYNC_EPI
        RPN4_EPI_STAGE(0); RPN4_EPI_STORE(0);
        RPN4_EPI_STAGE(1); RPN4_EPI_STORE(1);
        RPN4_EPI_STAGE(2); RPN4_EPI_STORE(2);
        RPN4_EPI_STAGE(3); RPN4_EPI_STORE(3);
        if constexpr (!POOL) {
            RPN4_EPI_STAGE(4); RPN4_EPI_STORE(4);
            RPN4_EPI_STAGE(5); RPN4_EPI_STORE(5);
            RPN4_EPI_STAGE(6); RPN4_EPI_STORE(6);
            RPN4_EPI_STAGE(7); RPN4_EPI_STORE(7);
        }
        pending = false;
#endif
        if (nxt < 0) break;
        cur = nxt; img = nimg; oy0 = noy0; ox0 = nox0; n0 = nn0;
        gt -= total_taps;
    }
    asm volatile("s_waitcnt vmcnt(0)" ::: "memory");
    if (pending) {
        RPN4_EPI_STAGE(0); RPN4_EPI_STORE(0);
        RPN4_EPI_STAGE(1); RPN4_EPI_STORE(1);
        RPN4_EPI_STAGE(2); RPN4_EPI_STORE(2);
        RPN4_EPI_STAGE(3); RPN4_EPI_STORE(3);
        if constexpr (!POOL) {
            RPN4_EPI_STAGE(4); RPN4_EPI_STORE(4);
            RPN4_EPI_STAGE(5); RPN4_EPI_STORE(5);
            RPN4_EPI_STAGE(6); RPN4_EPI_STORE(6);
            RPN4_EPI_STAGE(7); RPN4_EPI_STORE(7);
        }
    }
#undef RPN4_ROW_MFMA
#undef RPN4_EPI_STORE
#undef RPN4_EPI_STAGE
#undef RPN4_X_ADDR
#undef RPN4_W_ADDR
#undef RPN4_DMA_A
#undef RPN4_DMA_B
#undef halo_goff4
}
#endif

static inline unsigned short f32_to_bf16_rne(float f);
static inline float bf16_to_f32(unsigned short h);

template <bool F16, bool OUT_SPLIT, int STRIDE, int NTILES>
__global__ void __launch_bounds__(256)
conv_cin3_mfma_kernel(const float *__restrict__ x, const uint4 *__restrict__ w ,
                      const float *__restrict__ bias, void *__restrict__ out, int B, int H, int W, int OH, int OW,
                      int pad_t, int pad_l, int act, float out_scale, int tiles_x, int tiles_y, unsigned *status)
{
    constexpr int COUT = 16 * NTILES;
    constexpr int PR = 7 * STRIDE + 3, PC = 31 * STRIDE + 3;
    constexpr int PATCH = PR * PC * 3;
    constexpr int STAGE_LD = COUT + kStagePad;
    __shared__ __attribute__((aligned(16))) float patch[(PATCH + 3) / 4 * 4];
    __shared__ uint4 wl[COUT * 8];
    __shared__ __attribute__((aligned(16))) float stage_all[4 * 32 * STAGE_LD];

    const int tid = threadIdx.x, lane = tid & 63, wave = tid >> 6;
    const int lr = lane & 15, kg = lane >> 4;
    int t = blockIdx.x;
    const int tx = t % tiles_x;
    t /= tiles_x;
    const int ty = t % tiles_y;
    const int img = t / tiles_y;
    const int oy0 = ty * 8, ox0 = tx * 32;
    const int iy0 = oy0 * STRIDE - pad_t, ix0 = ox0 * STRIDE - pad_l;
    const float *ximg = x + (size_t)img * H * W * 3;

    for (int e = tid; e < PATCH; e += 256) {
        const int pr = e / (PC * 3), rem = e - pr * (PC * 3);
        const int iy = iy0 + pr, ix = ix0 + rem / 3;
        patch[e] = (iy >= 0 && iy < H && ix >= 0 && ix < W) ? ximg[((size_t)iy * W + ix) * 3 + rem % 3] : 0.0f;
    }
    for (int e = tid; e < COUT * 8; e += 256) {
        const int n = e >> 3, pc = e & 7;
        reinterpret_cast<u32x4 *>(wl)[n * 8 + (pc ^ ((n >> 1) & 7))] = reinterpret_cast<const u32x4 *>(w)[e];
    }
    int koff[8];
#pragma unroll
    for (int j = 0; j < 8; ++j) {
        const int k = 8 * kg + j;
        koff[j] = k < 27 ? (k / 9) * (PC * 3) + (k % 9) : -1;
    }
    __syncthreads();

    u32x4 bhi[NTILES], blo[NTILES];
#pragma unroll
    for (int j = 0; j < NTILES; ++j) {
        const int n = j * 16 + lr;
        const int idx = n * 8 + (kg ^ ((n >> 1) & 7));
        bhi[j] = reinterpret_cast<const u32x4 *>(wl)[idx];
        blo[j] = reinterpret_cast<const u32x4 *>(wl)[idx ^ 4];
    }
    f32x4 acc[4][NTILES];
#pragma unroll
    for (int m = 0; m < 4; ++m) {
        const int prow = (2 * wave + (m >> 1)) * STRIDE, pcol = (16 * (m & 1) + lr) * STRIDE;
        const int base = (prow * PC + pcol) * 3;
        float xs[8];
#pragma unroll
        for (int j = 0; j < 8; ++j) xs[j] = koff[j] >= 0 ? patch[base + koff[j]] : 0.0f;
        const u32x4 ahi = __builtin_bit_cast(u32x4, split_piece<F16>(xs, false));
        const u32x4 alo = __builtin_bit_cast(u32x4, split_piece<F16>(xs, true));
#pragma unroll
        for (int j = 0; j < NTILES; ++j) {
            f32x4 c = f32x4{0.f, 0.f, 0.f, 0.f};
            c = mfma16<F16>(alo, bhi[j], c);
            c = mfma16<F16>(ahi, blo[j], c);
            acc[m][j] = mfma16<F16>(ahi, bhi[j], c);
        }
    }

    float *stage = stage_all + wave * (32 * STAGE_LD);
    float bias_v[NTILES];
#pragma unroll
    for (int j = 0; j < NTILES; ++j) bias_v[j] = bias ? bias[j * 16 + lr] : 0.0f;
    const float act_lo = act == ACT_LINEAR ? -INFINITY : 0.0f;
    const float act_hi = act == ACT_RELU6 ? 6.0f : INFINITY;
    constexpr int PPX = COUT / 4;
#pragma unroll
    for (int i = 0; i < 2; ++i) {
#pragma unroll
        for (int hf = 0; hf < 2; ++hf)
#pragma unroll
            for (int j = 0; j < NTILES; ++j)
#pragma unroll
                for (int r = 0; r < 4; ++r)
                    stage[(16 * hf + 4 * kg + r) * STAGE_LD + j * 16 + lr] =
                        fminf(fmaxf(acc[i * 2 + hf][j][r] * out_scale + bias_v[j], act_lo), act_hi);
        __syncthreads();
        const int oy = oy0 + 2 * wave + i;
        if (oy < OH) {
            for (int e = lane; e < 32 * PPX; e += 64) {
                const int px = e / PPX, q = e - px * PPX;
                const int ox = ox0 + px;
                if (ox >= OW) continue;
                const size_t pix = ((size_t)img * OH + oy) * OW + ox;
                if constexpr (OUT_SPLIT) {
                    const int cl = q >> 2, pc = q & 3;
                    float xs[8];
                    const float *src = &stage[px * STAGE_LD + cl * 16 + (pc >> 1) * 8];
                    const float4 v0 = *reinterpret_cast<const float4 *>(src);
                    const float4 v1 = *reinterpret_cast<const float4 *>(src + 4);
                    xs[0] = v0.x; xs[1] = v0.y; xs[2] = v0.z; xs[3] = v0.w;
                    xs[4] = v1.x; xs[5] = v1.y; xs[6] = v1.z; xs[7] = v1.w;
                    reinterpret_cast<uint4 *>(out)[pix * PPX + q] = split_piece<F16>(xs, (pc & 1) != 0, status);
                } else {
                    reinterpret_cast<float4 *>(out)[pix * PPX + q] =
                        *reinterpret_cast<const float4 *>(&stage[px * STAGE_LD + 4 * q]);
                }
            }
        }
        __syncthreads();
    }
}

void pack_weights_cin3_mfma_host(const float *hwio, const float *scale, int Cout, int cout_pad, bool f16, int shift,
                                 unsigned short *dst )
{
    const float mul = ldexpf(1.0f, shift);
    memset(dst, 0, (size_t)cout_pad * 64 * sizeof(unsigned short));
    for (int k = 0; k < 27; ++k)
        for (int n = 0; n < Cout; ++n) {
            float v = hwio[(size_t)k * Cout + n];
            if (scale) v *= scale[n];
            v *= mul;
            unsigned short hi, lo;
            if (f16) {
                const _Float16 h = (_Float16)v;
                const _Float16 l = (_Float16)(v - (float)h);
                memcpy(&hi, &h, 2);
                memcpy(&lo, &l, 2);
            } else {
                hi = f32_to_bf16_rne(v);
                lo = f32_to_bf16_rne(v - bf16_to_f32(hi));
            }
            unsigned short *rec = dst + (size_t)n * 64;
            rec[(k >> 3) * 8 + (k & 7)] = hi;
            rec[(4 + (k >> 3)) * 8 + (k & 7)] = lo;
        }
}

hipError_t launch_conv_cin3_mfma(const float *x, const void *w, const float *bias, void *out, int B, int H, int W,
                                 int OH, int OW, int Cout, int stride, int pad_t, int pad_l, int act, float out_scale,
                                 int out_fmt, bool f16, hipStream_t s)
{
    if ((Cout != 32 && Cout != 64) || (stride != 1 && stride != 2) || act == ACT_SIGMOID) return hipErrorInvalidValue;
    const int tiles_x = (OW + 31) / 32, tiles_y = (OH + 7) / 8;
    const long long nblocks = (long long)tiles_x * tiles_y * B;
    if (nblocks <= 0 || nblocks > 0x7fffffffll) return hipErrorInvalidValue;
#define RPN_C3M(F16_, SPLIT_, STRIDE_, NT_)                                                                          \
    hipLaunchKernelGGL((conv_cin3_mfma_kernel<F16_, SPLIT_, STRIDE_, NT_>), dim3((unsigned)nblocks), dim3(256), 0, s, x, \
                       (const uint4 *)w, bias, out, B, H, W, OH, OW, pad_t, pad_l, act, out_scale, tiles_x, tiles_y, range_status())
#define RPN_C3M_FMT(F16_, STRIDE_, NT_) \
    { if (out_fmt) RPN_C3M(F16_, true, STRIDE_, NT_); else RPN_C3M(F16_, false, STRIDE_, NT_); }
#define RPN_C3M_ST(F16_, NT_) \
    { if (stride == 1) RPN_C3M_FMT(F16_, 1, NT_) else RPN_C3M_FMT(F16_, 2, NT_) }
    if (f16) { if (Cout == 64) RPN_C3M_ST(true, 4) else RPN_C3M_ST(true, 2) }
    else     { if (Cout == 64) RPN_C3M_ST(false, 4) else RPN_C3M_ST(false, 2) }
#undef RPN_C3M_ST
#undef RPN_C3M_FMT
#undef RPN_C3M
    return hipGetLastError();
}

template <bool F16>
__global__ void __launch_bounds__(256)
f32_to_split_kernel(const float *__restrict__ x, long long npieces, uint4 *__restrict__ out, unsigned *status)
{
    for (long long p = (long long)blockIdx.x * 256 + threadIdx.x; p < npieces; p += (long long)gridDim.x * 256) {
        const long long rec = p >> 2;
        const int pc = (int)(p & 3);
        const float *src = x + rec * 16 + (pc >> 1) * 8;
        const float4 v0 = *reinterpret_cast<const float4 *>(src);
        const float4 v1 = *reinterpret_cast<const float4 *>(src + 4);
        const float xs[8] = {v0.x, v0.y, v0.z, v0.w, v1.x, v1.y, v1.z, v1.w};
        out[p] = split_piece<F16>(xs, (pc & 1) != 0, status);
    }
}

template <bool F16>
__global__ void __launch_bounds__(256)
split_to_f32_kernel(const uint4 *__restrict__ x, long long nhalf, float *__restrict__ out)
{
    for (long long p = (long long)blockIdx.x * 256 + threadIdx.x; p < nhalf; p += (long long)gridDim.x * 256) {
        const uint4 hi = x[2 * p], lo = x[2 * p + 1];
        const unsigned h[4] = {hi.x, hi.y, hi.z, hi.w}, l[4] = {lo.x, lo.y, lo.z, lo.w};
        float o[8];
#pragma unroll
        for (int k = 0; k < 4; ++k) {
            o[2 * k] = join<F16>((unsigned short)(h[k] & 0xffffu), (unsigned short)(l[k] & 0xffffu));
            o[2 * k + 1] = join<F16>((unsigned short)(h[k] >> 16), (unsigned short)(l[k] >> 16));
        }
        float4 *dst = reinterpret_cast<float4 *>(out + p * 8);
        dst[0] = make_float4(o[0], o[1], o[2], o[3]);
        dst[1] = make_float4(o[4], o[5], o[6], o[7]);
    }
}

template <bool F16>
__global__ void __launch_bounds__(256)
maxpool_split_kernel(const uint4 *__restrict__ x, int H, int W, int G, int OH, int OW, long long total,
                     uint4 *__restrict__ out)
{
    for (long long i = (long long)blockIdx.x * 256 + threadIdx.x; i < total; i += (long long)gridDim.x * 256) {
        const int g = (int)(i % G);
        long long t = i / G;
        const int ox = (int)(t % OW);
        t /= OW;
        const int oy = (int)(t % OH);
        const long long b = t / OH;
        unsigned bh[4] = {0, 0, 0, 0}, bl[4] = {0, 0, 0, 0};
        float best[8];
#pragma unroll
        for (int dy = 0; dy < 2; ++dy)
#pragma unroll
            for (int dx = 0; dx < 2; ++dx) {
                const size_t pix = ((size_t)b * H + 2 * oy + dy) * W + 2 * ox + dx;
                const uint4 hi = x[(pix * G + g) * 2], lo = x[(pix * G + g) * 2 + 1];
                const unsigned h[4] = {hi.x, hi.y, hi.z, hi.w}, l[4] = {lo.x, lo.y, lo.z, lo.w};
#pragma unroll
                for (int k = 0; k < 8; ++k) {
                    const unsigned short hs = (unsigned short)((k & 1) ? (h[k >> 1] >> 16) : (h[k >> 1] & 0xffffu));
                    const unsigned short ls = (unsigned short)((k & 1) ? (l[k >> 1] >> 16) : (l[k >> 1] & 0xffffu));
                    const float v = join<F16>(hs, ls);
                    if ((dy == 0 && dx == 0) || v > best[k]) {
                        best[k] = v;
                        const unsigned sh = (k & 1) ? 16u : 0u;
                        const unsigned m = 0xffffu << sh;
                        bh[k >> 1] = (bh[k >> 1] & ~m) | ((unsigned)hs << sh);
                        bl[k >> 1] = (bl[k >> 1] & ~m) | ((unsigned)ls << sh);
                    }
                }
            }
        const size_t opix = ((size_t)b * OH + oy) * OW + ox;
        out[(opix * G + g) * 2] = make_uint4(bh[0], bh[1], bh[2], bh[3]);
        out[(opix * G + g) * 2 + 1] = make_uint4(bl[0], bl[1], bl[2], bl[3]);
    }
}

struct __attribute__((packed, aligned(4))) F4u {
    float x, y, z, w;
};

template <bool F16, bool OUT_SPLIT, int STRIDE, bool WCG = false>
__global__ void __launch_bounds__(256)
conv_cin3_kernel(const float *__restrict__ x, const float *__restrict__ w ,
                 const float *__restrict__ bias, void *__restrict__ out, int B, int H, int W, int OH, int OW,
                 int Cout, int stride, int pad_t, int pad_l, int act, long long npairs, unsigned *status)
{
    extern __shared__ __attribute__((aligned(16))) float wl[];
    const int CG = Cout >> 4;
    uint4 *stage = reinterpret_cast<uint4 *>(WCG ? wl : wl + 28 * Cout);
    if constexpr (!WCG) {
        for (int i = threadIdx.x; i < 27 * Cout; i += 256) wl[i] = w[i];
        for (int i = threadIdx.x; i < Cout; i += 256) wl[27 * Cout + i] = bias ? bias[i] : 0.0f;
        __syncthreads();
    }
    const int PW = (OW + 1) >> 1;
    const int pairs_per_block = 256 / CG;
    const unsigned pair0 = blockIdx.x * (unsigned)pairs_per_block;
    const unsigned row0 = pair0 / (unsigned)PW;
    const int x0 = (int)(pair0 - row0 * (unsigned)PW);
    const int wv = __builtin_amdgcn_readfirstlane((int)threadIdx.x >> 6);
    const int cg = WCG ? wv % CG : (int)threadIdx.x % CG;
    const int pairl = WCG ? ((int)threadIdx.x & 63) + 64 * (wv / CG) : (int)threadIdx.x / CG;
    const bool live = pair0 + (unsigned)pairl < (unsigned)npairs;
    int px2 = x0 + pairl;
    unsigned rowf = row0;
    while (px2 >= PW) {
        px2 -= PW;
        ++rowf;
    }
    const int img = (int)(rowf / (unsigned)OH);
    const int oy = (int)(rowf - (unsigned)img * (unsigned)OH);
    const int ox = 2 * px2;
    (void)stride;

    using f2 = __attribute__((ext_vector_type(2))) float;
    f2 acc[2][8];
#pragma unroll
    for (int n = 0; n < 8; ++n) {
        if constexpr (WCG) acc[0][n] = bias ? f2{bias[cg * 16 + 2 * n], bias[cg * 16 + 2 * n + 1]} : f2{0.0f, 0.0f};
        else acc[0][n] = f2{wl[27 * Cout + cg * 16 + 2 * n], wl[27 * Cout + cg * 16 + 2 * n + 1]};
        acc[1][n] = acc[0][n];
    }
    if (live) {
        const float *ximg = x + (size_t)img * H * W * 3;
        const int c0 = ox * STRIDE - pad_l;
        float win3[WCG ? 3 : 1][16];
        if constexpr (WCG) {
            const int iy0 = oy * STRIDE - pad_t;
            if (iy0 >= 0 && iy0 + 2 < H && c0 >= 0 && c0 * 3 + 16 <= W * 3) {
#pragma unroll
                for (int r = 0; r < 3; ++r) {
                    const F4u *src = reinterpret_cast<const F4u *>(ximg + ((size_t)(iy0 + r) * W + c0) * 3);
#pragma unroll
                    for (int v4 = 0; v4 < 4; ++v4) {
                        const F4u v = src[v4];
                        win3[r][4 * v4] = v.x; win3[r][4 * v4 + 1] = v.y; win3[r][4 * v4 + 2] = v.z; win3[r][4 * v4 + 3] = v.w;
                    }
                }
            } else {
#pragma unroll
                for (int r = 0; r < 3; ++r) {
                    const int iy = iy0 + r;
                    const bool row_ok = iy >= 0 && iy < H;
#pragma unroll
                    for (int j = 0; j < 15; ++j) {
                        const int col = c0 + j / 3;
                        const bool v = row_ok && col >= 0 && col < W && j < 3 * (STRIDE + 3);
                        win3[r][j] = v ? ximg[((size_t)iy * W + col) * 3 + j % 3] : 0.0f;
                    }
                    win3[r][15] = 0.0f;
                }
            }
        }
#pragma unroll(WCG ? 3 : 1)
        for (int r = 0; r < 3; ++r) {
            const int iy = oy * STRIDE + r - pad_t;
            const bool row_ok = iy >= 0 && iy < H;
            float win[16];
            if constexpr (WCG) {
#pragma unroll
                for (int j = 0; j < 16; ++j) win[j] = win3[r][j];
            } else if (row_ok && c0 >= 0 && c0 * 3 + 16 <= W * 3) {
                const F4u *src = reinterpret_cast<const F4u *>(ximg + ((size_t)iy * W + c0) * 3);
#pragma unroll
                for (int v4 = 0; v4 < 4; ++v4) {
                    const F4u v = src[v4];
                    win[4 * v4] = v.x; win[4 * v4 + 1] = v.y; win[4 * v4 + 2] = v.z; win[4 * v4 + 3] = v.w;
                }
            } else {
#pragma unroll
                for (int j = 0; j < 15; ++j) {
                    const int col = c0 + j / 3;
                    const bool v = row_ok && col >= 0 && col < W && j < 3 * (STRIDE + 3);
                    win[j] = v ? ximg[((size_t)iy * W + col) * 3 + j % 3] : 0.0f;
                }
                win[15] = 0.0f;
            }
#pragma unroll
            for (int sc = 0; sc < 9; ++sc) {
                const float4 *wk = WCG ? reinterpret_cast<const float4 *>(w + (r * 9 + sc) * Cout + cg * 16)
                                       : reinterpret_cast<const float4 *>(&wl[(r * 9 + sc) * Cout + cg * 16]);
                const float4 w0 = wk[0], w1 = wk[1], w2 = wk[2], w3 = wk[3];
                const f2 ws[8] = {{w0.x, w0.y}, {w0.z, w0.w}, {w1.x, w1.y}, {w1.z, w1.w},
                                  {w2.x, w2.y}, {w2.z, w2.w}, {w3.x, w3.y}, {w3.z, w3.w}};
                const float in0 = win[sc], in1 = win[sc + 3 * STRIDE];
                const f2 i0 = {in0, in0}, i1 = {in1, in1};
#pragma unroll
                for (int n = 0; n < 8; ++n) {
                    acc[0][n] = __builtin_elementwise_fma(i0, ws[n], acc[0][n]);
                    acc[1][n] = __builtin_elementwise_fma(i1, ws[n], acc[1][n]);
                }
            }
        }
    }
    const float act_lo = act == ACT_LINEAR ? -INFINITY : 0.0f;
    const float act_hi = act == ACT_RELU6 ? 6.0f : INFINITY;
#pragma unroll
    for (int p = 0; p < 2; ++p) {
        float v[16];
#pragma unroll
        for (int n = 0; n < 16; ++n) v[n] = fminf(fmaxf(acc[p][n >> 1][n & 1], act_lo), act_hi);
        uint4 *dst = stage + (2 * pairl + p) * (4 * CG);
        const int q0 = 4 * cg, sw = WCG ? (pairl & (4 * CG - 1) & 7) : 0;
        if constexpr (OUT_SPLIT) {
            const float lo8[8] = {v[0], v[1], v[2], v[3], v[4], v[5], v[6], v[7]};
            const float hi8[8] = {v[8], v[9], v[10], v[11], v[12], v[13], v[14], v[15]};
            dst[(q0 + 0) ^ sw] = split_piece<F16>(lo8, false, status);
            dst[(q0 + 1) ^ sw] = split_piece<F16>(lo8, true);
            dst[(q0 + 2) ^ sw] = split_piece<F16>(hi8, false, status);
            dst[(q0 + 3) ^ sw] = split_piece<F16>(hi8, true);
        } else {
#pragma unroll
            for (int k = 0; k < 4; ++k)
                dst[(q0 + k) ^ sw] = make_uint4(__float_as_uint(v[4 * k]), __float_as_uint(v[4 * k + 1]),
                                                __float_as_uint(v[4 * k + 2]), __float_as_uint(v[4 * k + 3]));
        }
    }
    __syncthreads();
    const int ppp = 4 * CG;
    const int total = 2 * pairs_per_block * ppp;
    uint4 *gout = reinterpret_cast<uint4 *>(out);
    for (int e = threadIdx.x; e < total; e += 256) {
        const int pl = e / ppp, q = e - pl * ppp;
        if (pair0 + (unsigned)(pl >> 1) >= (unsigned)npairs) continue;
        int gx2 = x0 + (pl >> 1);
        unsigned grow = row0;
        while (gx2 >= PW) {
            gx2 -= PW;
            ++grow;
        }
        const int gox = 2 * gx2 + (pl & 1);
        if (gox >= OW) continue;
        gout[((size_t)grow * OW + gox) * ppp + q] = stage[WCG ? pl * ppp + (q ^ ((pl >> 1) & (ppp - 1) & 7)) : e];
    }
}

constexpr int kC3Rows = 8;
constexpr int kC3PatchRow = 200;
constexpr int kC3Stage = ((kC3Rows + 2) * 198 + 255) / 256;
constexpr int kC3PatchFloats = (kC3Stage * 256 / 198 + 1) * kC3PatchRow;
struct C3Tile {
    int img, by, bx;
};
template <bool RELU>
__global__ void __launch_bounds__(256, 2)
conv_cin3_f32_mfma_kernel(const float *__restrict__ x, const float *__restrict__ w , const float *__restrict__ bias,
                          float *__restrict__ out, int H, int W, int tiles_x, int tiles_y, int n_tiles)
{
    __shared__ float patch[2][kC3PatchFloats];
    const int tid = threadIdx.x, lane = tid & 63;
    const int wv = __builtin_amdgcn_readfirstlane(tid >> 6);
    const int px = lane & 15, kq = lane >> 4;
    constexpr unsigned kOob = 0x80000000u;
    float aw[7][4];
#pragma unroll
    for (int kk = 0; kk < 7; ++kk) {
        const int k = 4 * kk + kq;
#pragma unroll
        for (int nb = 0; nb < 4; ++nb) {
            const float v = w[(k < 27 ? k : 26) * 64 + nb * 16 + px];
            aw[kk][nb] = k < 27 ? v : 0.0f;
        }
    }
    f32x4 bv[4];
#pragma unroll
    for (int nb = 0; nb < 4; ++nb) bv[nb] = f32x4{0.0f, 0.0f, 0.0f, 0.0f};
    if (bias) {
#pragma unroll
        for (int nb = 0; nb < 4; ++nb)
#pragma unroll
            for (int i = 0; i < 4; ++i) bv[nb][i] = bias[nb * 16 + 4 * kq + i];
    }
    int rd[7];
#pragma unroll
    for (int kk = 0; kk < 7; ++kk) {
        const int e = 4 * kk + kq < 27 ? 4 * kk + kq : 26, r = e / 9, t = e - 9 * r;
        rd[kk] = (wv + r) * kC3PatchRow + 3 * px + t;
    }
    int st_lds[kC3Stage];
    unsigned st_off[kC3Stage];
#pragma unroll
    for (int it = 0; it < kC3Stage; ++it) {
        const int i = tid + 256 * it, r = i / 198, j = i - 198 * r;
        st_lds[it] = r * kC3PatchRow + j;
        st_off[it] = r < kC3Rows + 2 ? (unsigned)((r * W * 3 + j) * 4) : kOob;
    }
    const int tiles_xy = tiles_x * tiles_y;
    const int g = (int)gridDim.x, d_img = g / tiles_xy, d_by = (g - d_img * tiles_xy) / tiles_x, d_bx = g - d_img * tiles_xy - d_by * tiles_x;
    auto advance = [&](C3Tile t) {
        t.bx += d_bx;
        if (t.bx >= tiles_x) {
            t.bx -= tiles_x;
            ++t.by;
        }
        t.by += d_by;
        if (t.by >= tiles_y) {
            t.by -= tiles_y;
            ++t.img;
        }
        t.img += d_img;
        return t;
    };
    float pre[kC3Stage];
    auto request = [&](C3Tile t) {
        const __amdgpu_buffer_rsrc_t in_rs = __builtin_amdgcn_make_buffer_rsrc(const_cast<float *>(x) + (size_t)t.img * H * W * 3, (short)0,
                                                                               H * W * 12, 0x00020000);
        if (t.by >= 1 && t.by * kC3Rows + kC3Rows + 1 <= H && t.bx >= 1 && t.bx * 192 + 195 <= 3 * W) {
            const int tbase = (((t.by * kC3Rows - 1) * W * 3) + t.bx * 192 - 3) * 4;
#pragma unroll
            for (int it = 0; it < kC3Stage; ++it)
                pre[it] = __builtin_bit_cast(float, __builtin_amdgcn_raw_buffer_load_b32(in_rs, st_off[it], tbase, 0));
        } else {
#pragma unroll
            for (int it = 0; it < kC3Stage; ++it) {
                const int i = tid + 256 * it, r = i / 198, j = i - 198 * r;
                const int iy = t.by * kC3Rows - 1 + r, fx = t.bx * 192 - 3 + j;
                const bool ok = r < kC3Rows + 2 && iy >= 0 && iy < H && fx >= 0 && fx < 3 * W;
                pre[it] = __builtin_bit_cast(float, __builtin_amdgcn_raw_buffer_load_b32(in_rs, ok ? (unsigned)((iy * W * 3 + fx) * 4) : kOob, 0, 0));
            }
        }
    };
    auto deposit = [&](int buf) {
#pragma unroll
        for (int it = 0; it < kC3Stage; ++it) patch[buf][st_lds[it]] = pre[it];
    };
    const unsigned st_out = (unsigned)((px * 64 + 4 * kq) * 4);
    int tile = blockIdx.x, buf = 0;
    C3Tile cur;
    cur.img = tile / tiles_xy;
    cur.by = (tile - cur.img * tiles_xy) / tiles_x;
    cur.bx = tile - cur.img * tiles_xy - cur.by * tiles_x;
    if (tile < n_tiles) {
        request(cur);
        deposit(0);
    }
    __syncthreads();
    for (; tile < n_tiles; tile += g, buf ^= 1) {
        const bool more = tile + g < n_tiles;
        C3Tile nxt = advance(cur);
        if (!more) nxt.by = -0x100000;
        const int x0 = cur.bx * 64;
        const bool whole = x0 + 64 <= W;
        const __amdgpu_buffer_rsrc_t out_rs = __builtin_amdgcn_make_buffer_rsrc(out + (size_t)cur.img * H * W * 64, (short)0, H * W * 256,
                                                                                0x00020000);
        float pin[4][7];
#pragma unroll
        for (int mb = 0; mb < 4; ++mb)
#pragma unroll
            for (int kk = 0; kk < 7; ++kk) pin[mb][kk] = patch[buf][rd[kk] + mb * 48];
        request(nxt);
#pragma unroll
        for (int h = 0; h < 2; ++h) {
            const int y = cur.by * kC3Rows + wv + 4 * h;
            const bool row = y < H;
            const int tb = (y * W + x0) * 256;
            if (h == 1) {
#pragma unroll
                for (int mb = 0; mb < 4; ++mb)
#pragma unroll
                    for (int kk = 0; kk < 7; ++kk) pin[mb][kk] = patch[buf][4 * kC3PatchRow + rd[kk] + mb * 48];
            }
#pragma unroll
            for (int mb = 0; mb < 4; ++mb) {
                f32x4 acc[4];
#pragma unroll
                for (int nb = 0; nb < 4; ++nb) acc[nb] = bv[nb];
#pragma unroll
                for (int kk = 0; kk < 7; ++kk)
#pragma unroll
                    for (int nb = 0; nb < 4; ++nb) acc[nb] = __builtin_amdgcn_mfma_f32_16x16x4f32(aw[kk][nb], pin[mb][kk], acc[nb], 0, 0, 0);
                if constexpr (RELU) {
#pragma unroll
                    for (int nb = 0; nb < 4; ++nb)
#pragma unroll
                        for (int i = 0; i < 4; ++i) {
                            const float f = acc[nb][i];
                            acc[nb][i] = __int_as_float(__builtin_elementwise_max(__float_as_int(f), 0));
                        }
                }
                const unsigned vo = (row && (whole || x0 + 16 * mb + px < W)) ? st_out + (unsigned)(tb + mb * 4096) : kOob;
#pragma unroll
                for (int nb = 0; nb < 4; ++nb)
                    __builtin_amdgcn_raw_buffer_store_b128(__builtin_bit_cast(u32x4, acc[nb]), out_rs, vo + (unsigned)(nb * 64), 0, 0);
            }
        }
        deposit(buf ^ 1);
        cur = nxt;
        __syncthreads();
    }
}

bool conv_cin3_uses_f32_mfma(int B, int H, int W, int OH, int OW, int Cout, int stride, int pad_t, int pad_l, int act, int out_fmt)
{
    static const int f32_mfma = RPN_LAB_KNOB("RPN_CIN3_F32_MFMA", 1);
    return f32_mfma && out_fmt == 0 && Cout == 64 && stride == 1 && pad_t == 1 && pad_l == 1 && OH == H && OW == W &&
           (act == ACT_RELU || act == ACT_LINEAR) && (long long)H * W * 256 < 0x7fffffffll && B > 0 && H > 0 && W > 0 &&
           (long long)((W + 63) / 64) * ((H + 7) / 8) * B < 0x7fffffffll;
}

hipError_t launch_conv_cin3(const float *x, const float *w, const float *bias, void *out, int B, int H, int W,
                            int OH, int OW, int Cout, int stride, int pad_t, int pad_l, int act, int out_fmt, bool f16,
                            hipStream_t s)
{
    if (Cout % 16 != 0 || Cout > 256 || 256 % (Cout / 16) != 0 || act == ACT_SIGMOID) return hipErrorInvalidValue;
    if (conv_cin3_uses_f32_mfma(B, H, W, OH, OW, Cout, stride, pad_t, pad_l, act, out_fmt)) {
        const int tiles_x = (W + 63) / 64, tiles_y = (H + kC3Rows - 1) / kC3Rows;
        const long long n_tiles = (long long)tiles_x * tiles_y * B;
        if (n_tiles >= 0x7fffffffll) return hipErrorInvalidValue;
        int dev = 0, n_cus = 0;
        if (hipGetDevice(&dev) != hipSuccess || hipDeviceGetAttribute(&n_cus, hipDeviceAttributeMultiprocessorCount, dev) != hipSuccess ||
            n_cus < 1)
            n_cus = 256;
        const dim3 grid((unsigned)(n_tiles < 3ll * n_cus ? n_tiles : 3ll * n_cus));
        if (act == ACT_RELU)
            hipLaunchKernelGGL(conv_cin3_f32_mfma_kernel<true>, grid, dim3(256), 0, s, x, w, bias, static_cast<float *>(out), H, W,
                               tiles_x, tiles_y, (int)n_tiles);
        else
            hipLaunchKernelGGL(conv_cin3_f32_mfma_kernel<false>, grid, dim3(256), 0, s, x, w, bias, static_cast<float *>(out), H, W,
                               tiles_x, tiles_y, (int)n_tiles);
        return hipGetLastError();
    }
    const long long npairs = (long long)B * OH * ((OW + 1) / 2);
    const long long threads = npairs * (Cout / 16);
    if (threads <= 0) return hipSuccess;
    if (npairs >= 0x7fffffffll || threads / 256 >= 0x7fffffffll) return hipErrorInvalidValue;
    const unsigned grid = (unsigned)((threads + 255) / 256);
    const bool wcg = Cout <= 64 && 4 % (Cout / 16) == 0;
    const size_t lds = (wcg ? 0 : (size_t)28 * Cout * sizeof(float)) + (size_t)2048 * 16;
#define RPN_CIN3(F16_, SPLIT_, STRIDE_)                                                                       \
    do {                                                                                                      \
        if (wcg)                                                                                              \
            hipLaunchKernelGGL((conv_cin3_kernel<F16_, SPLIT_, STRIDE_, true>), dim3(grid), dim3(256), lds, s, x, w, bias, out, B, \
                               H, W, OH, OW, Cout, stride, pad_t, pad_l, act, npairs, range_status());         \
        else                                                                                                  \
            hipLaunchKernelGGL((conv_cin3_kernel<F16_, SPLIT_, STRIDE_, false>), dim3(grid), dim3(256), lds, s, x, w, bias, out, B, \
                               H, W, OH, OW, Cout, stride, pad_t, pad_l, act, npairs, range_status());         \
    } while (0)
    if (stride != 1 && stride != 2) return hipErrorInvalidValue;
    if (out_fmt == 0) {
        if (stride == 1) RPN_CIN3(false, false, 1); else RPN_CIN3(false, false, 2);
    } else if (f16) {
        if (stride == 1) RPN_CIN3(true, true, 1); else RPN_CIN3(true, true, 2);
    } else {
        if (stride == 1) RPN_CIN3(false, true, 1); else RPN_CIN3(false, true, 2);
    }
#undef RPN_CIN3
    return hipGetLastError();
}

static thread_local unsigned *t_range_status = nullptr;
void set_range_status(unsigned *p) { t_range_status = p; }
unsigned *range_status() { return t_range_status; }

static inline unsigned short f32_to_bf16_rne(float f)
{
    unsigned u;
    memcpy(&u, &f, 4);
    if ((u & 0x7fffffffu) > 0x7f800000u) return (unsigned short)((u >> 16) | 0x40u);
    u += 0x7fffu + ((u >> 16) & 1u);
    return (unsigned short)(u >> 16);
}
static inline float bf16_to_f32(unsigned short h)
{
    const unsigned u = (unsigned)h << 16;
    float f;
    memcpy(&f, &u, 4);
    return f;
}

int split_weight_shift(const float *hwio, size_t count, bool f16)
{
    if (!f16) return 0;
    float mx = 0.0f;
    for (size_t i = 0; i < count; ++i) {
        const float v = hwio[i] < 0 ? -hwio[i] : hwio[i];
        if (v > mx) mx = v;
    }
    if (!(mx > 0.0f)) return 0;
    int e = 0;
    (void)frexpf(mx, &e);
    int s = 12 - e;
    if (s < -100) s = -100;
    if (s > 24) s = 24;
    return s;
}

void pack_weights_split_host(const float *hwio, const float *scale, int Cin, int Cout, int cout_pad, bool f16,
                             int shift, unsigned short *dst )
{
    const int chunks = Cin / 16;
    const float mul = ldexpf(1.0f, shift);
    memset(dst, 0, (size_t)9 * chunks * cout_pad * 32 * sizeof(unsigned short));
    for (int t = 0; t < 9; ++t)
        for (int c = 0; c < Cin; ++c)
            for (int n = 0; n < Cout; ++n) {
                float v = hwio[((size_t)t * Cin + c) * Cout + n];
                if (scale) v *= scale[n];
                v *= mul;
                unsigned short hi, lo;
                if (f16) {
                    const _Float16 h = (_Float16)v;
                    const _Float16 l = (_Float16)(v - (float)h);
                    memcpy(&hi, &h, 2);
                    memcpy(&lo, &l, 2);
                } else {
                    hi = f32_to_bf16_rne(v);
                    lo = f32_to_bf16_rne(v - bf16_to_f32(hi));
                }
                const int chunk = c >> 4, g = (c >> 3) & 1, k = c & 7;
                unsigned short *rec = dst + (((size_t)chunk * 9 + t) * cout_pad + n) * 32;
                rec[(g * 2 + 0) * 8 + k] = hi;
                rec[(g * 2 + 1) * 8 + k] = lo;
            }
}

void pack_weights_split32_host(const float *hwio, const float *scale, int Cin, int Cout, int cout_pad, bool f16,
                               int shift, unsigned short *dst )
{
    const int chunks = Cin / 32;
    const float mul = ldexpf(1.0f, shift);
    memset(dst, 0, (size_t)9 * chunks * cout_pad * 64 * sizeof(unsigned short));
    for (int t = 0; t < 9; ++t)
        for (int c = 0; c < Cin; ++c)
            for (int n = 0; n < Cout; ++n) {
                float v = hwio[((size_t)t * Cin + c) * Cout + n];
                if (scale) v *= scale[n];
                v *= mul;
                unsigned short hi, lo;
                if (f16) {
                    const _Float16 h = (_Float16)v;
                    const _Float16 l = (_Float16)(v - (float)h);
                    memcpy(&hi, &h, 2);
                    memcpy(&lo, &l, 2);
                } else {
                    hi = f32_to_bf16_rne(v);
                    lo = f32_to_bf16_rne(v - bf16_to_f32(hi));
                }
                const int chunk = c >> 5, kgq = (c >> 3) & 3, k = c & 7;
                unsigned short *rec = dst + (((size_t)chunk * 9 + t) * cout_pad + n) * 64;
                const int swz = (n >> 1) & 7;
                rec[(kgq ^ swz) * 8 + k] = hi;
                rec[((4 + kgq) ^ swz) * 8 + k] = lo;
            }
}

static int grid_cap(long long items)
{
    long long g = (items + 255) / 256;
    if (g < 1) g = 1;
    if (g > 8192) g = 8192;
    return (int)g;
}

hipError_t launch_f32_to_split(const float *x, long long npix, int C, bool f16, void *out, hipStream_t s)
{
    if (C % 16 != 0) return hipErrorInvalidValue;
    const long long pieces = npix * (C / 16) * 4;
    if (pieces == 0) return hipSuccess;
    if (f16) hipLaunchKernelGGL(f32_to_split_kernel<true>, dim3(grid_cap(pieces)), dim3(256), 0, s, x, pieces, (uint4 *)out, range_status());
    else hipLaunchKernelGGL(f32_to_split_kernel<false>, dim3(grid_cap(pieces)), dim3(256), 0, s, x, pieces, (uint4 *)out, range_status());
    return hipGetLastError();
}

hipError_t launch_split_to_f32(const void *x, long long npix, int C, bool f16, float *out, hipStream_t s)
{
    if (C % 16 != 0) return hipErrorInvalidValue;
    const long long halves = npix * (C / 8);
    if (halves == 0) return hipSuccess;
    if (f16) hipLaunchKernelGGL(split_to_f32_kernel<true>, dim3(grid_cap(halves)), dim3(256), 0, s, (const uint4 *)x, halves, out);
    else hipLaunchKernelGGL(split_to_f32_kernel<false>, dim3(grid_cap(halves)), dim3(256), 0, s, (const uint4 *)x, halves, out);
    return hipGetLastError();
}

hipError_t launch_maxpool_split(const void *x, int B, int H, int W, int C, bool f16, void *out, hipStream_t s)
{
    if (C % 16 != 0) return hipErrorInvalidValue;
    const int OH = H / 2, OW = W / 2, G = C / 8;
    const long long total = (long long)B * OH * OW * G;
    if (total == 0) return hipSuccess;
    if (f16) hipLaunchKernelGGL(maxpool_split_kernel<true>, dim3(grid_cap(total)), dim3(256), 0, s, (const uint4 *)x, H, W, G, OH, OW, total, (uint4 *)out);
    else hipLaunchKernelGGL(maxpool_split_kernel<false>, dim3(grid_cap(total)), dim3(256), 0, s, (const uint4 *)x, H, W, G, OH, OW, total, (uint4 *)out);
    return hipGetLastError();
}

template <int TH, int WN, int BBUF, bool F16, bool POOL, int NW = 4>
static hipError_t launch_split_variant(const SplitConvArgs &a, hipStream_t s)
{
    constexpr int BN = (NW == 8 ? WN * 64 : WN * 64);
    const int tiles_x = (a.W + TWS - 1) / TWS, tiles_y = (a.H + TH - 1) / TH;
    const int n_tiles = (a.Cout + BN - 1) / BN;
    const long long m_tiles = (long long)tiles_x * tiles_y * a.B;
    const int XN = n_tiles >= 8 ? 8 : (n_tiles >= 4 ? 4 : (n_tiles >= 2 ? 2 : 1)), XM = 8 / XN;
    const long long nblocks = 8ll * ((n_tiles + XN - 1) / XN) * ((m_tiles + XM - 1) / XM);
    if (m_tiles <= 0 || nblocks > 0x7fffffffll) return hipErrorInvalidValue;
    hipLaunchKernelGGL((conv3x3_split_kernel<TH, WN, BBUF, NW, F16, POOL>), dim3((unsigned)nblocks), dim3(64 * NW), 0,
                       s, a, tiles_x, tiles_y, n_tiles);
    return hipGetLastError();
}


template <bool F16, bool POOL>
static hipError_t launch_split_tiles(const SplitConvArgs &a, hipStream_t s)
{
    static const int force_tile = RPN_LAB_KNOB("RPN_SPLIT_TILE", 0), force_bbuf = RPN_LAB_KNOB("RPN_SPLIT_BBUF", 0);
    const long long mt8 = (long long)((a.W + 31) / 32) * ((a.H + 7) / 8) * a.B;
    const long long mt4 = (long long)((a.W + 31) / 32) * ((a.H + 3) / 4) * a.B;
    const int nt128 = (a.Cout + 127) / 128;
    int tile;
    if (a.Cout <= 64) tile = 81;
    else if (mt8 * nt128 >= 512) tile = 82;
    else if (mt4 * nt128 >= 512 || POOL) tile = 42;
    else tile = 41;
    if (force_tile && a.Cout > 64 && !(POOL && force_tile == 41)) tile = force_tile;
    int bbuf = (tile == 82) ? 1 : 2;
    if (force_bbuf) bbuf = force_bbuf;
    if (tile == 82 && bbuf == 2) bbuf = 1;
    static const int force_waves = RPN_LAB_KNOB("RPN_SPLIT_WAVES", 0);
    if (tile == 82 && force_waves == 8) return launch_split_variant<8, 2, 1, F16, POOL, 8>(a, s);
    static const int small_mode = RPN_LAB_KNOB("RPN_SPLIT_SMALL", 0);
    if constexpr (!POOL) {
        if (tile == 41 && small_mode == 2 && mt4 * nt128 >= 256) return launch_split_variant<4, 2, 2, F16, false, 8>(a, s);
    }
    switch (tile * 10 + bbuf) {
        case 821: return launch_split_variant<8, 2, 1, F16, POOL>(a, s);
        case 811: return launch_split_variant<8, 1, 1, F16, POOL>(a, s);
        case 812: return launch_split_variant<8, 1, 2, F16, POOL>(a, s);
        case 421: return launch_split_variant<4, 2, 1, F16, POOL>(a, s);
        case 422: return launch_split_variant<4, 2, 2, F16, POOL>(a, s);
        case 411: if constexpr (!POOL) return launch_split_variant<4, 1, 1, F16, false>(a, s); else break;
        case 412: if constexpr (!POOL) return launch_split_variant<4, 1, 2, F16, false>(a, s); else break;
        default: break;
    }
    return hipErrorInvalidValue;
}

static unsigned *sched_counters(hipStream_t s)
{
    static const int dyn = RPN_KNOB("RPN_S16_DYN", 0);
    if (!dyn) return nullptr;
    static std::mutex mu;
    static std::unordered_map<hipStream_t, unsigned *> pool;
    std::lock_guard<std::mutex> lock(mu);
    auto it = pool.find(s);
    if (it != pool.end()) return it->second;
    hipStreamCaptureStatus st = hipStreamCaptureStatusNone;
    if (hipStreamIsCapturing(s, &st) != hipSuccess || st != hipStreamCaptureStatusNone) return nullptr;
    unsigned *p = nullptr;
    if (hipMalloc(&p, 128) != hipSuccess || hipMemset(p, 0, 128) != hipSuccess) {
        (void)hipGetLastError();
        return nullptr;
    }
    pool[s] = p;
    return p;
}

const char *conv3x3_split16_variant(int B, int H, int W, int Cin, int Cout, int cout_pad, bool pool)
{
    if (Cin % 32 != 0 || Cout % 16 != 0 || cout_pad % 64 != 0 || cout_pad < Cout) return nullptr;
    static const int dma_mode = RPN_LAB_KNOB("RPN_S16_DMA", 1);
    const long long big_blocks = (long long)((W + 31) / 32) * ((H + 7) / 8) * B * ((Cout + 127) / 128);
    const bool dma_ok = dma_mode && Cin % 64 == 0 && (long long)B * H * W * Cin * 4 < 0x7fffffffll &&
                        (long long)(Cin / 32) * 9 * cout_pad * 128 < 0x7fffffffll;
    const long long blocks64 = (long long)((W + 31) / 32) * ((H + 7) / 8) * B * ((Cout + 63) / 64);
    if (dma_ok && !pool && cout_pad % 128 == 0 && blocks64 <= 128) return "reg,64";
    if (dma_ok) return (cout_pad % 128 != 0 || big_blocks < 256) ? "dma,64" : "dma,128";
    if (cout_pad % 128 != 0) return nullptr;
    return (big_blocks < 256 && !pool) ? "reg,64" : "reg,128";
}

hipError_t launch_conv3x3_split16(const void *x, const void *w, const float *bias, void *out, int B, int H, int W,
                                  int Cin, int Cout, int cout_pad, float out_scale, int act, bool out_f32, bool f16,
                                  bool pool, hipStream_t s, bool ktree)
{
    if (Cin % 32 != 0 || Cout % 16 != 0 || cout_pad % 64 != 0 || act == ACT_SIGMOID) return hipErrorInvalidValue;
    if (ktree && (pool || !conv3x3_split16_ktree_ok(B, H, W, Cin, Cout, cout_pad))) return hipErrorInvalidValue;
    SplitConvArgs a{};
    a.status = range_status();
    a.x = (const uint4 *)x; a.w = (const uint4 *)w; a.bias = bias; a.out = out;
    a.B = B; a.H = H; a.W = W; a.Cin = Cin; a.Cout = Cout; a.cout_pad = cout_pad;
    a.out_scale = out_scale; a.act = act; a.out_f32 = out_f32 ? 1 : 0;
    const char *variant = ktree ? "dma,64" : conv3x3_split16_variant(B, H, W, Cin, Cout, cout_pad, pool);
    if (!variant) return hipErrorInvalidValue;
    a.ktree = ktree ? 1 : 0;
    const long long big_blocks = (long long)((W + 31) / 32) * ((H + 7) / 8) * B * ((Cout + 127) / 128);
    if (variant[0] == 'd') {
        const int BN = variant[4] == '6' ? 64 : 128;
        const int tiles_x = (W + TWS - 1) / TWS, tiles_y = (H + 7) / 8;
        const int n_tiles = (Cout + BN - 1) / BN;
        const long long m_tiles = (long long)tiles_x * tiles_y * B;
        const int XN = n_tiles >= 8 ? 8 : (n_tiles >= 4 ? 4 : (n_tiles >= 2 ? 2 : 1)), XM = 8 / XN;
        const long long slots = (long long)((n_tiles + XN - 1) / XN) * ((m_tiles + XM - 1) / XM);
        if (m_tiles <= 0 || slots > 0x0fffffffll) return hipErrorInvalidValue;
        static const int n_cus = [] {
            int dev = 0, n = 0;
            if (hipGetDevice(&dev) != hipSuccess ||
                hipDeviceGetAttribute(&n, hipDeviceAttributeMultiprocessorCount, dev) != hipSuccess || n < 8)
                n = 256;
            return n;
        }();
        const unsigned pgrid = 8u * (unsigned)(slots < n_cus / 8 ? slots : n_cus / 8);
        a.sched = sched_counters(s);
#define RPN_L16D(F16_, POOL_, BN_)                                                                                   \
    hipLaunchKernelGGL((conv3x3_split16_dma_kernel<F16_, POOL_, BN_>), dim3(pgrid), dim3(512), 0, s, a, tiles_x, tiles_y, \
                       n_tiles)
#define RPN_L16D_BN(F16_, POOL_)                                                                                     \
    if (BN == 128) RPN_L16D(F16_, POOL_, 128); else RPN_L16D(F16_, POOL_, 64)
#ifdef RPN_LAB
        static const int w4 = RPN_LAB_KNOB("RPN_S16_W4", 0);
        const long long out_bytes4 = (long long)B * (pool ? H >> 1 : H) * (pool ? W >> 1 : W) * Cout * 4;
        if (BN == 128 && (w4 == 1 || w4 == Cin) && !a.sched && out_bytes4 < 0x7fffffffll) {
#define RPN_L16D4(F16_, POOL_)                                                                                       \
    hipLaunchKernelGGL((conv3x3_split16_dma4_kernel<F16_, POOL_>), dim3(pgrid), dim3(256), 0, s, a, tiles_x, tiles_y, n_tiles)
            if (f16) { if (pool) { RPN_L16D4(true, true); } else { RPN_L16D4(true, false); } }
            else { if (pool) { RPN_L16D4(false, true); } else { RPN_L16D4(false, false); } }
#undef RPN_L16D4
            return hipGetLastError();
        }
#endif
        if (ktree) {
            if (f16) hipLaunchKernelGGL((conv3x3_split16_dma_kernel<true, false, 64, true>), dim3(pgrid), dim3(512), 0, s, a, tiles_x, tiles_y, n_tiles);
            else hipLaunchKernelGGL((conv3x3_split16_dma_kernel<false, false, 64, true>), dim3(pgrid), dim3(512), 0, s, a, tiles_x, tiles_y, n_tiles);
        } else if (f16) { if (pool) { RPN_L16D_BN(true, true); } else { RPN_L16D_BN(true, false); } }
        else { if (pool) { RPN_L16D_BN(false, true); } else { RPN_L16D_BN(false, false); } }
#undef RPN_L16D_BN
#undef RPN_L16D
        return hipGetLastError();
    }
    const bool small = big_blocks < 256 && !pool;
    const int TH = small ? 4 : 8, BN = small ? 64 : 128;
    const int tiles_x = (W + TWS - 1) / TWS, tiles_y = (H + TH - 1) / TH;
    const int n_tiles = (Cout + BN - 1) / BN;
    const long long m_tiles = (long long)tiles_x * tiles_y * B;
    const int XN = n_tiles >= 8 ? 8 : (n_tiles >= 4 ? 4 : (n_tiles >= 2 ? 2 : 1)), XM = 8 / XN;
    const long long nblocks = 8ll * ((n_tiles + XN - 1) / XN) * ((m_tiles + XM - 1) / XM);
    if (m_tiles <= 0 || nblocks > 0x7fffffffll) return hipErrorInvalidValue;
#define RPN_L16(TH_, WN_, NW_, F16_, POOL_)                                                                          \
    hipLaunchKernelGGL((conv3x3_split16_kernel<TH_, WN_, NW_, F16_, POOL_>), dim3((unsigned)nblocks), dim3(64 * NW_), 0, s, \
                       a, tiles_x, tiles_y, n_tiles)
    if (small) {
        if (f16) RPN_L16(4, 1, 4, true, false); else RPN_L16(4, 1, 4, false, false);
    } else if (f16) {
        if (pool) RPN_L16(8, 2, 8, true, true); else RPN_L16(8, 2, 8, true, false);
    } else {
        if (pool) RPN_L16(8, 2, 8, false, true); else RPN_L16(8, 2, 8, false, false);
    }
#undef RPN_L16
    return hipGetLastError();
}

bool conv3x3_split16_ktree_ok(int B, int H, int W, int Cin, int Cout, int cout_pad)
{
    static const int on = RPN_KNOB("RPN_KSPLIT", 1);
    return on && Cin % 64 == 0 && Cin >= 256 && Cout % 16 == 0 && cout_pad % 128 == 0 && cout_pad >= Cout &&
           (long long)B * H * W * Cin * 4 < 0x7fffffffll && (long long)(Cin / 32) * 9 * cout_pad * 128 < 0x7fffffffll;
}

bool conv3x3_split16_ksplit_dma(int B, int H, int W, int Cin, int Cout, int cout_pad)
{
    static const int on = RPN_LAB_KNOB("RPN_KSPLIT_DMA", 1);
    const char *v = conv3x3_split16_variant(B, H, W, Cin, Cout, cout_pad, false);
    if (!on || !v || strcmp(v, "reg,64") != 0) return false;
    const long long blocks64 = (long long)((W + 31) / 32) * ((H + 7) / 8) * B * ((Cout + 63) / 64);
    const int chunks = Cin / 32, mid = ktree_cut(chunks, 2);
    const int n_tiles = (Cout + 63) / 64;
    const long long m_tiles = (long long)((W + 31) / 32) * ((H + 7) / 8) * B;
    const int XN = n_tiles >= 8 ? 8 : (n_tiles >= 4 ? 4 : (n_tiles >= 2 ? 2 : 1)), XM = 8 / XN;
    const long long slots = (long long)((n_tiles + XN - 1) / XN) * ((m_tiles + XM - 1) / XM);
    return blocks64 > 64 && blocks64 <= 128 && slots <= 16 && mid >= 2 && (chunks - mid) >= 2 && (chunks - mid) % 2 == 0;
}

int conv3x3_split16_ksplit(int B, int H, int W, int Cin, int Cout, int cout_pad)
{
    if (conv3x3_split16_ksplit_dma(B, H, W, Cin, Cout, cout_pad)) return 2;
    const char *v = conv3x3_split16_variant(B, H, W, Cin, Cout, cout_pad, false);
    if (!v || strcmp(v, "reg,64") != 0) return 1;
    const long long blocks = (long long)((W + 31) / 32) * ((H + 3) / 4) * B * ((Cout + 63) / 64);
    const int chunks = Cin / 32;
    (void)chunks;
    return blocks <= 128 ? 4 : (blocks <= 256 ? 2 : 1);
}

hipError_t launch_conv3x3_split16_ksplit(const void *x, const void *w, float *out, long long slab_floats, int B, int H, int W,
                                         int Cin, int Cout, int cout_pad, float out_scale, bool f16, int ksplit, hipStream_t s)
{
    if ((ksplit != 2 && ksplit != 4) || !conv3x3_split16_ktree_ok(B, H, W, Cin, Cout, cout_pad)) return hipErrorInvalidValue;
    SplitConvArgs a{};
    a.status = nullptr;
    a.ktree = 1;
    a.x = (const uint4 *)x; a.w = (const uint4 *)w; a.bias = nullptr; a.out = out;
    a.B = B; a.H = H; a.W = W; a.Cin = Cin; a.Cout = Cout; a.cout_pad = cout_pad;
    a.out_scale = out_scale; a.act = ACT_LINEAR; a.out_f32 = 1; a.slab_floats = slab_floats;
    if (ksplit == 2 && conv3x3_split16_ksplit_dma(B, H, W, Cin, Cout, cout_pad)) {
        const int tiles_x = (W + TWS - 1) / TWS, tiles_y = (H + 7) / 8, n_tiles = (Cout + 63) / 64;
        const long long m_tiles = (long long)tiles_x * tiles_y * B;
        const int XN = n_tiles >= 8 ? 8 : (n_tiles >= 4 ? 4 : (n_tiles >= 2 ? 2 : 1)), XM = 8 / XN;
        const long long slots = (long long)((n_tiles + XN - 1) / XN) * ((m_tiles + XM - 1) / XM);
        if (m_tiles <= 0 || slots > 16) return hipErrorInvalidValue;
        const unsigned pgrid = 8u * (unsigned)slots;
        a.sched = nullptr;
        if (f16) hipLaunchKernelGGL((conv3x3_split16_dma_kernel<true, false, 64, true>), dim3(pgrid, 2), dim3(512), 0, s, a, tiles_x, tiles_y, n_tiles);
        else hipLaunchKernelGGL((conv3x3_split16_dma_kernel<false, false, 64, true>), dim3(pgrid, 2), dim3(512), 0, s, a, tiles_x, tiles_y, n_tiles);
        return hipGetLastError();
    }
    const int tiles_x = (W + TWS - 1) / TWS, tiles_y = (H + 3) / 4;
    const int n_tiles = (Cout + 63) / 64;
    const long long m_tiles = (long long)tiles_x * tiles_y * B;
    const int XN = n_tiles >= 8 ? 8 : (n_tiles >= 4 ? 4 : (n_tiles >= 2 ? 2 : 1)), XM = 8 / XN;
    const long long nblocks = 8ll * ((n_tiles + XN - 1) / XN) * ((m_tiles + XM - 1) / XM);
    if (m_tiles <= 0 || nblocks > 0x7fffffffll) return hipErrorInvalidValue;
    const dim3 grid((unsigned)nblocks, (unsigned)ksplit);
    if (f16) hipLaunchKernelGGL((conv3x3_split16_kernel<4, 1, 4, true, false>), grid, dim3(256), 0, s, a, tiles_x, tiles_y, n_tiles);
    else hipLaunchKernelGGL((conv3x3_split16_kernel<4, 1, 4, false, false>), grid, dim3(256), 0, s, a, tiles_x, tiles_y, n_tiles);
    return hipGetLastError();
}

hipError_t launch_conv3x3_split(const void *x, const void *w, const float *bias, void *out, int B, int H, int W,
                                int Cin, int Cout, int cout_pad, float out_scale, int act, bool out_f32, bool f16,
                                bool pool, hipStream_t s, bool ktree)
{
    if (ktree) return hipErrorInvalidValue;
    if (Cin % 16 != 0 || Cout % 16 != 0 || cout_pad % 64 != 0 || act == ACT_SIGMOID) return hipErrorInvalidValue;
    SplitConvArgs a{};
    a.status = range_status();
    a.x = (const uint4 *)x; a.w = (const uint4 *)w; a.bias = bias; a.out = out;
    a.B = B; a.H = H; a.W = W; a.Cin = Cin; a.Cout = Cout; a.cout_pad = cout_pad;
    a.out_scale = out_scale; a.act = act; a.out_f32 = out_f32 ? 1 : 0;
    if (pool) return f16 ? launch_split_tiles<true, true>(a, s) : launch_split_tiles<false, true>(a, s);
    return f16 ? launch_split_tiles<true, false>(a, s) : launch_split_tiles<false, false>(a, s);
}

hipError_t launch_vgg_block1(const float *img, const void *w1, const float *b1, float scale1, const void *w2,
                             const float *b2, float scale2, void *out, int B, int H, int W, bool f16, hipStream_t s)
{
    if (B < 1 || H < 2 || W < 2) return hipErrorInvalidValue;
    SplitConvArgs a{};
    a.status = range_status();
    a.x = nullptr; a.w = (const uint4 *)w2; a.bias = b2; a.out = out;
    a.B = B; a.H = H; a.W = W; a.Cin = 64; a.Cout = 64; a.cout_pad = 64;
    a.out_scale = scale2; a.act = ACT_RELU; a.out_f32 = 0;
    a.img = img; a.w1 = (const uint4 *)w1; a.b1 = b1; a.scale1 = scale1;
    const int tiles_x = (W + TWS - 1) / TWS, tiles_y = (H + 7) / 8;
    const long long m_tiles = (long long)tiles_x * tiles_y * B;
    const long long nblocks = 8ll * ((m_tiles + 7) / 8);
    if (nblocks > 0x7fffffffll) return hipErrorInvalidValue;
    if (f16)
        hipLaunchKernelGGL((conv3x3_split_kernel<8, 1, 2, 4, true, true, true>), dim3((unsigned)nblocks), dim3(256), 0, s, a,
                           tiles_x, tiles_y, 1);
    else
        hipLaunchKernelGGL((conv3x3_split_kernel<8, 1, 2, 4, false, true, true>), dim3((unsigned)nblocks), dim3(256), 0, s, a,
                           tiles_x, tiles_y, 1);
    return hipGetLastError();
}

}
```

Before: 3049 images/s.

## Add dedicated VGG block1 fused kernel with direct-to-LDS weight DMA pipeline

Moves the fused conv1_1+conv1_2+pool block out of the generic split-conv kernel into its own kernel. Weights for conv1_2 are streamed with buffer_load-to-LDS into a 3-slot ring, and the MFMA loop is fully unrolled over 36 steps with explicit sched_group_barriers that interleave LDS reads with MFMAs. The conv1_1 result is computed into LDS in two channel halves, using 16x16 MFMAs and the split hi/lo representation, instead of being recomputed per chunk inside the generic pipeline. Shared helpers move to a common header. This adds a lot of hand-scheduled code and specialised LDS layout assumptions, and the kernel is tied to fixed shapes.

```diff
diff --git a/tf_rpn_amd/csrc/conv_block1_kernels.hip b/tf_rpn_amd/csrc/conv_block1_kernels.hip
--- /dev/null
+++ b/tf_rpn_amd/csrc/conv_block1_kernels.hip
@@ -0,0 +1,293 @@
+#include "conv_split_common.h"
+
+namespace rpn {
+
+#define RPN_LDS_PTR(p) ((__attribute__((address_space(3))) void *)(p))
+
+__device__ __forceinline__ int b1_swz(int hx) { return (hx >> 1) & 7; }
+
+template <bool F16>
+__global__ void __launch_bounds__(256, 2)
+vgg_block1_dma_kernel(SplitConvArgs a, int tiles_x, int tiles_y)
+{
+    constexpr int TH = 8, NW = 4, RW = 2, NI = 2, PPP = 8, NSTEPS = 36;
+    constexpr int HP = (TH + 2) * HW;
+    constexpr int ABUF = (HP * PPP + 63) / 64 * 64;
+    constexpr int BSLOT = 64 * 4;
+    constexpr int PW = TWS + 4;
+    constexpr int PATCH_F = (TH + 4) * PW * 3;
+    constexpr int B_AT = ABUF, P_AT = B_AT + 3 * BSLOT;
+    constexpr int LDS_UINT4 = P_AT + (PATCH_F + 3) / 4;
+    constexpr int NBLK = (HP + 15) / 16;
+    constexpr int QB = (NBLK + NW - 1) / NW;
+    constexpr int STAGE_LD = 64 + kStagePad;
+    static_assert(NW * 32 * STAGE_LD <= ABUF * 4 && LDS_UINT4 * 16 <= 80 * 1024 && HP * PPP + PPP <= ABUF,
+                  "LDS map");
+
+    __shared__ uint4 lds[LDS_UINT4];
+    u32x4 *As = reinterpret_cast<u32x4 *>(lds);
+    u32x4 *Bs = As + B_AT;
+    float *patchf = reinterpret_cast<float *>(lds + P_AT);
+
+    const int tid = threadIdx.x;
+    const int lane = tid & 63;
+    const int wave = __builtin_amdgcn_readfirstlane(tid >> 6);
+    const int wm = wave;
+    const int lr = lane & 15, kg = lane >> 4;
+    const int lm = lane & 31, kh = lane >> 5;
+
+    int t = blockIdx.x;
+    const int tx = t % tiles_x;
+    t /= tiles_x;
+    const int ty = t % tiles_y;
+    const int img = t / tiles_y;
+    const int oy0 = ty * TH, ox0 = tx * TWS;
+
+    const __amdgpu_buffer_rsrc_t wrsrc =
+        __builtin_amdgcn_make_buffer_rsrc(const_cast<uint4 *>(a.w), (short)0, NSTEPS * BSLOT * 16, 0x00020000);
+    unsigned b_voff;
+    {
+        const int e = wave * 64 + lane, n = e >> 2, pc = e & 3;
+        b_voff = (unsigned)((n * 4 + (pc ^ ((n >> 2) & 3))) * 16);
+    }
+#define RPN_B1_DMA_W(STEP, SLOT)                                                                                   \
+    {                                                                                                              \
+        u32x4 *dst_ = Bs + (SLOT) * BSLOT + wave * 64;                                                             \
+        __builtin_amdgcn_raw_ptr_buffer_load_lds(wrsrc, RPN_LDS_PTR(dst_), 16, b_voff, (STEP) * BSLOT * 16, 0, 0);   \
+    }
+
+    int a_off[3][2];
+#pragma unroll
+    for (int s3 = 0; s3 < 3; ++s3)
+#pragma unroll
+        for (int h16 = 0; h16 < 2; ++h16) {
+            const int hx = lm + s3;
+            a_off[s3][h16] = hx * PPP + ((2 * h16 + kh) ^ b1_swz(hx));
+        }
+    int b_off[NI];
+#pragma unroll
+    for (int j = 0; j < NI; ++j) {
+        const int n = j * 32 + lm;
+        b_off[j] = n * 4 + ((2 * kh) ^ ((n >> 2) & 3));
+    }
+#define RPN_X_ADDR(ROW, S, H16, I, LO) (As[(RW * wm + (ROW) + (I)) * HW * PPP + (a_off[S][H16] ^ ((LO) ? 4 : 0))])
+#define RPN_W_ADDR(SLOT, J, LO) (Bs[(SLOT) * BSLOT + (b_off[J] ^ ((LO) ? 1 : 0))])
+
+    int koff[8];
+#pragma unroll
+    for (int j = 0; j < 8; ++j) {
+        const int k = 8 * kg + j;
+        koff[j] = k < 27 ? (k / 9) * (PW * 3) + (k % 9) : -1;
+    }
+    float b1_max = 0.0f;
+#define RPN_B1_CONV1(C, UNROLL)                                                                                           \
+    {                                                                                                               \
+        u32x4 w1hi_[2], w1lo_[2];                                                                                   \
+        f32x4 b1v_[2];                                                                                              \
+        _Pragma("unroll") for (int h_ = 0; h_ < 2; ++h_) {                                                          \
+            const u32x4 *w1_ = reinterpret_cast<const u32x4 *>(a.w1) + (((C) * 2 + h_) * 16 + lr) * 8 + kg;        \
+            w1hi_[h_] = w1_[0];                                                                                     \
+            w1lo_[h_] = w1_[4];                                                                                     \
+            b1v_[h_] = *reinterpret_cast<const f32x4 *>(a.b1 + ((C) * 2 + h_) * 16 + 4 * kg);                        \
+        }                                                                                                           \
+        _Pragma(UNROLL) for (int q_ = 0; q_ < QB; ++q_) {                                                           \
+            const int p_ = (wave + NW * q_) * 16 + lr;                                                              \
+            const bool valid_ = p_ < HP;                                                                            \
+            const int pp_ = valid_ ? p_ : HP - 1;                                                                   \
+            const int hy_ = pp_ / HW, hx_ = pp_ - hy_ * HW;                                                         \
+            const int base_ = (hy_ * PW + hx_) * 3;                                                                 \
+            float xs_[8];                                                                                           \
+            _Pragma("unroll") for (int j_ = 0; j_ < 8; ++j_) xs_[j_] = koff[j_] >= 0 ? patchf[base_ + koff[j_]] : 0.0f; \
+            const u32x4 phi_ = __builtin_bit_cast(u32x4, split_piece<F16>(xs_, false));                             \
+            const u32x4 plo_ = __builtin_bit_cast(u32x4, split_piece<F16>(xs_, true));                              \
+            const int iy_ = oy0 - 1 + hy_, ix_ = ox0 - 1 + hx_;                                                     \
+            const bool in_ = valid_ && iy_ >= 0 && iy_ < a.H && ix_ >= 0 && ix_ < a.W;                               \
+            const int swz_ = b1_swz(hx_);                                                                           \
+            _Pragma("unroll") for (int h_ = 0; h_ < 2; ++h_) {                                                      \
+                f32x4 c_ = {0.f, 0.f, 0.f, 0.f};                                                                    \
+                c_ = mfma16<F16>(w1lo_[h_], phi_, c_);                                                              \
+                c_ = mfma16<F16>(w1hi_[h_], plo_, c_);                                                              \
+                c_ = mfma16<F16>(w1hi_[h_], phi_, c_);                                                              \
+                using E_ = typename Half<F16>::elem;                                                                \
+                using h4_ = __attribute__((ext_vector_type(4))) E_;                                                 \
+                h4_ hv_, lv_;                                                                                       \
+                _Pragma("unroll") for (int r_ = 0; r_ < 4; ++r_) {                                                  \
+                    float v_ = fmaxf(c_[r_] * a.scale1 + b1v_[h_][r_], 0.0f);                                       \
+                    v_ = in_ ? v_ : 0.0f;                                                                           \
+                    b1_max = fmaxf(b1_max, v_);                                                                     \
+                    const E_ e_ = (E_)v_;                                                                           \
+                    hv_[r_] = e_;                                                                                   \
+                    lv_[r_] = (E_)(v_ - (float)e_);                                                                 \
+                }                                                                                                   \
+                 \
+                const int dst_ = valid_ ? (pp_ * PPP + ((2 * h_ + (kg >> 1)) ^ swz_)) * 16 + (kg & 1) * 8          \
+                                        : (HP * PPP + 2 * h_ + (kg >> 1)) * 16 + (kg & 1) * 8;                       \
+                char *d_ = reinterpret_cast<char *>(As);                                                            \
+                *reinterpret_cast<uint2 *>(d_ + dst_) = __builtin_bit_cast(uint2, hv_);                             \
+                *reinterpret_cast<uint2 *>(d_ + (dst_ ^ 64)) = __builtin_bit_cast(uint2, lv_);                      \
+            }                                                                                                       \
+        }                                                                                                           \
+    }
+
+#pragma unroll
+    for (int tp = 0; tp < 3; ++tp) RPN_B1_DMA_W(tp, tp);
+    {
+        const float *ximg = a.img + (size_t)img * a.H * a.W * 3;
+        for (int e = tid; e < PATCH_F; e += 64 * NW) {
+            const int pr = e / (PW * 3), rem = e - pr * (PW * 3);
+            const int iy = oy0 - 2 + pr, ix = ox0 - 2 + rem / 3;
+            patchf[e] = (iy >= 0 && iy < a.H && ix >= 0 && ix < a.W) ? ximg[((size_t)iy * a.W + ix) * 3 + rem % 3] : 0.0f;
+        }
+    }
+    __syncthreads();
+    RPN_B1_CONV1(0, "unroll");
+    __syncthreads();
+
+    u32x4 fx0[2], fx1[2], fw[2][2 * NI];
+#pragma unroll
+    for (int i = 0; i < 2 * NI; ++i) fw[0][i] = RPN_W_ADDR(0, i >> 1, i & 1);
+#pragma unroll
+    for (int i = 0; i < 2; ++i) fx0[i] = RPN_X_ADDR(0, 0, 0, 0, i);
+    asm volatile("s_waitcnt lgkmcnt(0)" ::: "memory");
+    __builtin_amdgcn_s_barrier();
+
+    f32x16 acc[RW][NI];
+#pragma unroll
+    for (int i = 0; i < RW; ++i)
+#pragma unroll
+        for (int j = 0; j < NI; ++j)
+#pragma unroll
+            for (int e = 0; e < 16; ++e) acc[i][j][e] = 0.0f;
+
+#pragma unroll
+    for (int K = 0; K < NSTEPS; ++K) {
+        const int s9 = K % 9, H16 = (K / 9) & 1;
+        const int CS = K & 1, CR = s9 / 3, CC = s9 % 3;
+        const int NS = (K + 1) & 1, NH16 = ((K + 1) / 9) & 1, NR = ((K + 1) % 9) / 3, NC = ((K + 1) % 9) % 3;
+        const bool dma = K + 3 < NSTEPS;
+        const bool next_w = K + 1 < NSTEPS;
+        const bool next_x = next_w && K != 17;
+        if (dma) RPN_B1_DMA_W(K + 3, K % 3);
+#pragma unroll
+        for (int j = 0; j < NI; ++j) {
+            if (j == 0) { fx1[0] = RPN_X_ADDR(CR, CC, H16, 1, 0); fx1[1] = RPN_X_ADDR(CR, CC, H16, 1, 1); }
+            acc[0][j] = Half<F16>::mfma(fx0[1], fw[CS][2 * j], acc[0][j]);
+            acc[0][j] = Half<F16>::mfma(fx0[0], fw[CS][2 * j + 1], acc[0][j]);
+            acc[0][j] = Half<F16>::mfma(fx0[0], fw[CS][2 * j], acc[0][j]);
+        }
+        if (dma) __builtin_amdgcn_sched_group_barrier(0x020, 1, 0);
+#pragma unroll
+        for (int i = 0; i < 2; ++i) {
+            __builtin_amdgcn_sched_group_barrier(0x100, 1, 0);
+            __builtin_amdgcn_sched_group_barrier(0x008, 1, 0);
+        }
+        __builtin_amdgcn_sched_group_barrier(0x008, 3 * NI - 2, 0);
+        __builtin_amdgcn_sched_barrier(0);
+#pragma unroll
+        for (int j = 0; j < NI; ++j) {
+            if (next_w) { fw[NS][2 * j] = RPN_W_ADDR((K + 1) % 3, j, 0); fw[NS][2 * j + 1] = RPN_W_ADDR((K + 1) % 3, j, 1); }
+            acc[1][j] = Half<F16>::mfma(fx1[1], fw[CS][2 * j], acc[1][j]);
+            acc[1][j] = Half<F16>::mfma(fx1[0], fw[CS][2 * j + 1], acc[1][j]);
+            if (next_x && j == NI - 1) { fx0[0] = RPN_X_ADDR(NR, NC, NH16, 0, 0); fx0[1] = RPN_X_ADDR(NR, NC, NH16, 0, 1); }
+            acc[1][j] = Half<F16>::mfma(fx1[0], fw[CS][2 * j], acc[1][j]);
+        }
+        if (next_w) {
+#pragma unroll
+            for (int i = 0; i < 2 * NI; ++i) {
+                __builtin_amdgcn_sched_group_barrier(0x100, 1, 0);
+                __builtin_amdgcn_sched_group_barrier(0x008, 1, 0);
+            }
+        } else {
+            __builtin_amdgcn_sched_group_barrier(0x008, 2 * NI, 0);
+        }
+        if (next_x) {
+#pragma unroll
+            for (int i = 0; i < 2; ++i) {
+                __builtin_amdgcn_sched_group_barrier(0x100, 1, 0);
+                __builtin_amdgcn_sched_group_barrier(0x008, 1, 0);
+            }
+        } else {
+            __builtin_amdgcn_sched_group_barrier(0x008, 2, 0);
+        }
+        __builtin_amdgcn_sched_barrier(0);
+        if (dma) asm volatile("s_waitcnt vmcnt(1)" ::: "memory");
+        else asm volatile("s_waitcnt vmcnt(0)" ::: "memory");
+        asm volatile("s_waitcnt lgkmcnt(0)" ::: "memory");
+        __builtin_amdgcn_s_barrier();
+        __builtin_amdgcn_sched_barrier(0);
+        if (K == 17) {
+            RPN_B1_CONV1(1, "unroll 3");
+            __syncthreads();
+#pragma unroll
+            for (int i = 0; i < 2; ++i) fx0[i] = RPN_X_ADDR(0, 0, 0, 0, i);
+        }
+    }
+#undef RPN_B1_DMA_W
+#undef RPN_B1_CONV1
+#undef RPN_X_ADDR
+#undef RPN_W_ADDR
+    if constexpr (F16) {
+        if (a.status && !(b1_max <= 65504.0f)) atomicOr(a.status, 1u );
+    }
+
+    float *stage = reinterpret_cast<float *>(lds) + wave * (32 * STAGE_LD);
+    float bias_v[NI];
+#pragma unroll
+    for (int j = 0; j < NI; ++j) bias_v[j] = a.bias ? a.bias[j * 32 + lm] : 0.0f;
+#pragma unroll
+    for (int j = 0; j < NI; ++j)
+#pragma unroll
+        for (int e2 = 0; e2 < 8; ++e2) {
+            const float v0 = fmaxf(acc[0][j][2 * e2], acc[0][j][2 * e2 + 1]);
+            const float v1 = fmaxf(acc[1][j][2 * e2], acc[1][j][2 * e2 + 1]);
+            const int m2 = (e2 & 1) + 4 * (e2 >> 1) + 2 * kh;
+            stage[m2 * STAGE_LD + j * 32 + lm] = fminf(fmaxf(fmaxf(v0, v1) * a.out_scale + bias_v[j], 0.0f), INFINITY);
+        }
+    wave_sync();
+    const int OHo = a.H >> 1, OWo = a.W >> 1, oy = (oy0 + wm * RW) >> 1, oxb = ox0 >> 1;
+    if (oy < OHo) {
+        constexpr int pix_bytes = 4 * 64;
+        const long long row_off = (((long long)img * OHo + oy) * OWo + oxb) * (long long)pix_bytes;
+        const __amdgpu_buffer_rsrc_t ors = __builtin_amdgcn_make_buffer_rsrc(reinterpret_cast<char *>(a.out) + row_off, (short)0,
+                                                                              (OWo - oxb) * pix_bytes, 0x00020000);
+        const int px2 = lane >> 3, q2 = lane & 7;
+        const int cl = q2 >> 1, hf = q2 & 1;
+        unsigned voff = (unsigned)(px2 * pix_bytes + cl * 64 + hf * 32);
+#pragma unroll
+        for (int rd = 0; rd < 2; ++rd) {
+            float xs[8];
+            const float *src = &stage[(rd * 8 + px2) * STAGE_LD + cl * 16 + hf * 8];
+            const float4 v0 = *reinterpret_cast<const float4 *>(src);
+            const float4 v1 = *reinterpret_cast<const float4 *>(src + 4);
+            xs[0] = v0.x; xs[1] = v0.y; xs[2] = v0.z; xs[3] = v0.w;
+            xs[4] = v1.x; xs[5] = v1.y; xs[6] = v1.z; xs[7] = v1.w;
+            const u32x4 hi = __builtin_bit_cast(u32x4, split_piece<F16>(xs, false, a.status));
+            const u32x4 lo = __builtin_bit_cast(u32x4, split_piece<F16>(xs, true, nullptr));
+            __builtin_amdgcn_raw_buffer_store_b128(hi, ors, voff, 0, 0);
+            __builtin_amdgcn_raw_buffer_store_b128(lo, ors, voff + 16u, 0, 0);
+            voff += (unsigned)(8 * pix_bytes);
+        }
+    }
+}
+
+hipError_t launch_vgg_block1(const float *img, const void *w1, const float *b1, float scale1, const void *w2,
+                             const float *b2, float scale2, void *out, int B, int H, int W, bool f16, hipStream_t s)
+{
+    if (B < 1 || H < 2 || W < 2) return hipErrorInvalidValue;
+    SplitConvArgs a{};
+    a.status = range_status();
+    a.x = nullptr; a.w = (const uint4 *)w2; a.bias = b2; a.out = out;
+    a.B = B; a.H = H; a.W = W; a.Cin = 64; a.Cout = 64; a.cout_pad = 64;
+    a.out_scale = scale2; a.act = ACT_RELU; a.out_f32 = 0;
+    a.img = img; a.w1 = (const uint4 *)w1; a.b1 = b1; a.scale1 = scale1;
+    const int tiles_x = (W + TWS - 1) / TWS, tiles_y = (H + 7) / 8;
+    const long long nblocks = (long long)tiles_x * tiles_y * B;
+    if (nblocks > 0x7fffffffll) return hipErrorInvalidValue;
+    if (f16)
+        hipLaunchKernelGGL(vgg_block1_dma_kernel<true>, dim3((unsigned)nblocks), dim3(256), 0, s, a, tiles_x, tiles_y);
+    else
+        hipLaunchKernelGGL(vgg_block1_dma_kernel<false>, dim3((unsigned)nblocks), dim3(256), 0, s, a, tiles_x, tiles_y);
+    return hipGetLastError();
+}
+
+}
diff --git a/tf_rpn_amd/csrc/conv_split_common.h b/tf_rpn_amd/csrc/conv_split_common.h
--- /dev/null
+++ b/tf_rpn_amd/csrc/conv_split_common.h
@@ -0,0 +1,228 @@
+#pragma once
+
+#include "conv_kernels.h"
+
+#include <cmath>
+
+#ifndef RPN_STAMP_AT
+#define RPN_STAMP_AT(k) ((void)0)
+#endif
+
+namespace rpn {
+
+__device__ __forceinline__ void wave_sync()
+{
+    __builtin_amdgcn_fence(__ATOMIC_RELEASE, "wavefront");
+    __builtin_amdgcn_wave_barrier();
+    __builtin_amdgcn_fence(__ATOMIC_ACQUIRE, "wavefront");
+}
+
+using f32x16 = __attribute__((ext_vector_type(16))) float;
+using bf16x8 = __attribute__((ext_vector_type(8))) __bf16;
+using f16x8 = __attribute__((ext_vector_type(8))) _Float16;
+using u32x4 = __attribute__((ext_vector_type(4))) unsigned;
+
+constexpr int TWS = 32;
+constexpr int HW = TWS + 2;
+constexpr int kStagePad = 4;
+
+template <bool F16> struct Half;
+template <> struct Half<false> {
+    using vec = bf16x8;
+    using elem = __bf16;
+    static __device__ __forceinline__ f32x16 mfma(u32x4 a, u32x4 b, f32x16 c)
+    {
+        return __builtin_amdgcn_mfma_f32_32x32x16_bf16(__builtin_bit_cast(bf16x8, a), __builtin_bit_cast(bf16x8, b), c,
+                                                       0, 0, 0);
+    }
+};
+template <> struct Half<true> {
+    using vec = f16x8;
+    using elem = _Float16;
+    static __device__ __forceinline__ f32x16 mfma(u32x4 a, u32x4 b, f32x16 c)
+    {
+        return __builtin_amdgcn_mfma_f32_32x32x16_f16(__builtin_bit_cast(f16x8, a), __builtin_bit_cast(f16x8, b), c, 0,
+                                                      0, 0);
+    }
+};
+
+template <bool F16>
+__device__ __forceinline__ uint4 split_piece(const float (&x)[8], bool lo, unsigned *status = nullptr)
+{
+    using E = typename Half<F16>::elem;
+    typename Half<F16>::vec v;
+    if constexpr (F16) {
+        if (status && !lo) {
+            const float m = fmaxf(fmaxf(fmaxf(fabsf(x[0]), fabsf(x[1])), fmaxf(fabsf(x[2]), fabsf(x[3]))),
+                                  fmaxf(fmaxf(fabsf(x[4]), fabsf(x[5])), fmaxf(fabsf(x[6]), fabsf(x[7]))));
+            float nan_probe = 0.0f;
+#pragma unroll
+            for (int k = 0; k < 8; ++k) nan_probe = fmaf(x[k], 0.0f, nan_probe);
+            if (!(m <= 65504.0f) || nan_probe != 0.0f) atomicOr(status, 1u );
+        }
+    }
+#pragma unroll
+    for (int k = 0; k < 8; ++k) {
+        const E h = (E)x[k];
+        v[k] = lo ? (E)(x[k] - (float)h) : h;
+    }
+    return __builtin_bit_cast(uint4, v);
+}
+
+template <bool F16>
+__device__ __forceinline__ float join(unsigned short hi, unsigned short lo)
+{
+    using E = typename Half<F16>::elem;
+    return (float)__builtin_bit_cast(E, hi) + (float)__builtin_bit_cast(E, lo);
+}
+
+using f32x4 = __attribute__((ext_vector_type(4))) float;
+
+template <bool F16>
+__device__ __forceinline__ f32x4 mfma16(u32x4 a, u32x4 b, f32x4 c)
+{
+    if constexpr (F16)
+        return __builtin_amdgcn_mfma_f32_16x16x32_f16(__builtin_bit_cast(f16x8, a), __builtin_bit_cast(f16x8, b), c, 0, 0, 0);
+    else
+        return __builtin_amdgcn_mfma_f32_16x16x32_bf16(__builtin_bit_cast(bf16x8, a), __builtin_bit_cast(bf16x8, b), c, 0, 0, 0);
+}
+
+__device__ __forceinline__ int halo_swz(int hx) { return hx & 6; }
+
+__device__ __forceinline__ int xcd_remap_s(int bid, int nwg)
+{
+    const int q = nwg >> 3, r = nwg & 7, xcd = bid & 7;
+    return (xcd < r ? xcd * (q + 1) : r * (q + 1) + (xcd - r) * q) + (bid >> 3);
+}
+
+struct SplitConvArgs {
+    const uint4 *x;
+    const uint4 *w;
+    const float *bias;
+    void *out;
+    int B, H, W, Cin, Cout, cout_pad;
+    float out_scale;
+    int act, out_f32;
+    unsigned *sched;
+    unsigned *status;
+    const float *img;
+    const uint4 *w1;
+    const float *b1;
+    float scale1;
+    long long slab_floats;
+    int ktree;
+};
+
+template <bool F16, bool POOL, int RW, int NW, int NJ = 4>
+__device__ __forceinline__ void split16_epilogue(f32x4 (&acc)[RW * 2][NJ], float *lds_f, const SplitConvArgs &a, int img,
+                                                 int oy0, int ox0, int n0, int wave, int wm, int wn, int lane,
+                                                 int stamp_base = -1 )
+{
+    (void)stamp_base;
+    asm volatile("" : "+v"(lane));
+    constexpr int MT = RW * 2;
+    constexpr int CW = 16 * NJ;
+    constexpr int STAGE_LD = CW + kStagePad;
+    constexpr int PP = CW / 4;
+    const int lr = lane & 15, kg = lane >> 4;
+    float *stage = lds_f + wave * (32 * STAGE_LD);
+    float bias_v[NJ];
+#pragma unroll
+    for (int j = 0; j < NJ; ++j) {
+        const int n = n0 + wn * CW + j * 16 + lr;
+        bias_v[j] = (a.bias && n < a.Cout) ? a.bias[n] : 0.0f;
+    }
+    const float act_lo = a.act == ACT_LINEAR ? -INFINITY : 0.0f;
+    const float act_hi = a.act == ACT_RELU6 ? 6.0f : INFINITY;
+    const int cout_chunks = a.Cout >> 4;
+    const int nbase = n0 + wn * CW;
+    const int pix_bytes = a.out_f32 ? a.Cout * 4 : cout_chunks * 64;
+    constexpr int PXR = 64 / PP;
+    const int px_l = lane / PP, q_l = lane % PP;
+    auto store_stage = [&](int npx_log2, int oy, int oxb, int OHo, int OWo) {
+        if (oy >= OHo) return;
+        const int rounds = (PP << npx_log2) >> 6;
+        const long long row_off = (((long long)img * OHo + oy) * OWo + oxb) * (long long)pix_bytes;
+        const __amdgpu_buffer_rsrc_t ors = __builtin_amdgcn_make_buffer_rsrc(reinterpret_cast<char *>(a.out) + row_off, (short)0,
+                                                                              (OWo - oxb) * pix_bytes, 0x00020000);
+        if (a.out_f32) {
+            const int n = nbase + 4 * q_l;
+            unsigned voff = n < a.Cout ? (unsigned)(px_l * pix_bytes + n * 4) : 0x80000000u;
+#pragma unroll
+            for (int rd = 0; rd < rounds; ++rd) {
+                const u32x4 v = *reinterpret_cast<const u32x4 *>(&stage[(rd * PXR + px_l) * STAGE_LD + 4 * q_l]);
+#ifdef RPN_NOSTORE
+                __builtin_amdgcn_raw_buffer_store_b128(v, ors, (unsigned)(lane * 16), 0, 0);
+#else
+                __builtin_amdgcn_raw_buffer_store_b128(v, ors, voff, 0, 0);
+#endif
+                voff += (unsigned)(PXR * pix_bytes);
+            }
+        } else {
+            constexpr int LPP = CW / 8;
+            constexpr int PXR2 = 64 / LPP;
+            const int px2 = lane / LPP, q2 = lane % LPP;
+            const int cl = q2 >> 1, hf = q2 & 1;
+            const int n = nbase + cl * 16;
+            unsigned voff = n < a.Cout ? (unsigned)(px2 * pix_bytes + (n >> 4) * 64 + hf * 32) : 0x80000000u;
+            const int rounds2 = (1 << npx_log2) / PXR2;
+#pragma unroll
+            for (int rd = 0; rd < rounds2; ++rd) {
+                float xs[8];
+                const float *src = &stage[(rd * PXR2 + px2) * STAGE_LD + cl * 16 + hf * 8];
+                const float4 v0 = *reinterpret_cast<const float4 *>(src);
+                const float4 v1 = *reinterpret_cast<const float4 *>(src + 4);
+                xs[0] = v0.x; xs[1] = v0.y; xs[2] = v0.z; xs[3] = v0.w;
+                xs[4] = v1.x; xs[5] = v1.y; xs[6] = v1.z; xs[7] = v1.w;
+                const u32x4 hi = __builtin_bit_cast(u32x4, split_piece<F16>(xs, false, a.status));
+                const u32x4 lo = __builtin_bit_cast(u32x4, split_piece<F16>(xs, true, nullptr));
+#ifdef RPN_NOSTORE
+                __builtin_amdgcn_raw_buffer_store_b128(hi, ors, (unsigned)(lane * 32), 0, 0);
+                __builtin_amdgcn_raw_buffer_store_b128(lo, ors, (unsigned)(lane * 32 + 16), 0, 0);
+#else
+                __builtin_amdgcn_raw_buffer_store_b128(hi, ors, voff, 0, 0);
+                __builtin_amdgcn_raw_buffer_store_b128(lo, ors, voff + 16u, 0, 0);
+#endif
+                voff += (unsigned)(PXR2 * pix_bytes);
+            }
+        }
+    };
+
+    if constexpr (POOL) {
+        const int OHo = a.H >> 1, OWo = a.W >> 1;
+#pragma unroll
+        for (int hf = 0; hf < 2; ++hf)
+#pragma unroll
+            for (int j = 0; j < NJ; ++j)
+#pragma unroll
+                for (int r2 = 0; r2 < 2; ++r2) {
+                    const float v0 = fmaxf(acc[hf][j][2 * r2], acc[hf][j][2 * r2 + 1]);
+                    const float v1 = fmaxf(acc[(MT - 2) + hf][j][2 * r2], acc[(MT - 2) + hf][j][2 * r2 + 1]);
+                    const int px2 = 8 * hf + 2 * kg + r2;
+                    stage[px2 * STAGE_LD + j * 16 + lr] = fminf(fmaxf(fmaxf(v0, v1) * a.out_scale + bias_v[j], act_lo), act_hi);
+                }
+        wave_sync();
+        store_stage(4, (oy0 + 2 * wm) >> 1, ox0 >> 1, OHo, OWo);
+    } else {
+#pragma unroll
+        for (int i = 0; i < RW; ++i) {
+#pragma unroll
+            for (int hf = 0; hf < 2; ++hf)
+#pragma unroll
+                for (int j = 0; j < NJ; ++j)
+#pragma unroll
+                    for (int r = 0; r < 4; ++r) {
+                        const int px = 16 * hf + 4 * kg + r;
+                        stage[px * STAGE_LD + j * 16 + lr] =
+                            fminf(fmaxf(acc[i * 2 + hf][j][r] * a.out_scale + bias_v[j], act_lo), act_hi);
+                    }
+            wave_sync();
+            if (stamp_base >= 0) RPN_STAMP_AT(stamp_base + 2 * i);
+            store_stage(5, oy0 + RW * wm + i, ox0, a.H, a.W);
+            wave_sync();
+            if (stamp_base >= 0) RPN_STAMP_AT(stamp_base + 2 * i + 1);
+        }
+    }
+}
+
+}
diff --git a/tf_rpn_amd/csrc/conv_split_kernels.hip b/tf_rpn_amd/csrc/conv_split_kernels.hip
--- a/tf_rpn_amd/csrc/conv_split_kernels.hip
+++ b/tf_rpn_amd/csrc/conv_split_kernels.hip
@@ -35,112 +35,11 @@
 #define RPN_STAMP_VAL(k, v) ((void)0)
 #endif
 
+#include "conv_split_common.h"
+
 namespace rpn {
 
-__device__ __forceinline__ void wave_sync()
-{
-    __builtin_amdgcn_fence(__ATOMIC_RELEASE, "wavefront");
-    __builtin_amdgcn_wave_barrier();
-    __builtin_amdgcn_fence(__ATOMIC_ACQUIRE, "wavefront");
-}
-
-using f32x16 = __attribute__((ext_vector_type(16))) float;
-using bf16x8 = __attribute__((ext_vector_type(8))) __bf16;
-using f16x8 = __attribute__((ext_vector_type(8))) _Float16;
-using u32x4 = __attribute__((ext_vector_type(4))) unsigned;
-
-constexpr int TWS = 32;
-constexpr int HW = TWS + 2;
-constexpr int kStagePad = 4;
-
-template <bool F16> struct Half;
-template <> struct Half<false> {
-    using vec = bf16x8;
-    using elem = __bf16;
-    static __device__ __forceinline__ f32x16 mfma(u32x4 a, u32x4 b, f32x16 c)
-    {
-        return __builtin_amdgcn_mfma_f32_32x32x16_bf16(__builtin_bit_cast(bf16x8, a), __builtin_bit_cast(bf16x8, b), c,
-                                                       0, 0, 0);
-    }
-};
-template <> struct Half<true> {
-    using vec = f16x8;
-    using elem = _Float16;
-    static __device__ __forceinline__ f32x16 mfma(u32x4 a, u32x4 b, f32x16 c)
-    {
-        return __builtin_amdgcn_mfma_f32_32x32x16_f16(__builtin_bit_cast(f16x8, a), __builtin_bit_cast(f16x8, b), c, 0,
-                                                      0, 0);
-    }
-};
-
-template <bool F16>
-__device__ __forceinline__ uint4 split_piece(const float (&x)[8], bool lo, unsigned *status = nullptr)
-{
-    using E = typename Half<F16>::elem;
-    typename Half<F16>::vec v;
-    if constexpr (F16) {
-        if (status && !lo) {
-            const float m = fmaxf(fmaxf(fmaxf(fabsf(x[0]), fabsf(x[1])), fmaxf(fabsf(x[2]), fabsf(x[3]))),
-                                  fmaxf(fmaxf(fabsf(x[4]), fabsf(x[5])), fmaxf(fabsf(x[6]), fabsf(x[7]))));
-            float nan_probe = 0.0f;
-#pragma unroll
-            for (int k = 0; k < 8; ++k) nan_probe = fmaf(x[k], 0.0f, nan_probe);
-            if (!(m <= 65504.0f) || nan_probe != 0.0f) atomicOr(status, 1u );
-        }
-    }
-#pragma unroll
-    for (int k = 0; k < 8; ++k) {
-        const E h = (E)x[k];
-        v[k] = lo ? (E)(x[k] - (float)h) : h;
-    }
-    return __builtin_bit_cast(uint4, v);
-}
-
-template <bool F16>
-__device__ __forceinline__ float join(unsigned short hi, unsigned short lo)
-{
-    using E = typename Half<F16>::elem;
-    return (float)__builtin_bit_cast(E, hi) + (float)__builtin_bit_cast(E, lo);
-}
-
-using f32x4 = __attribute__((ext_vector_type(4))) float;
-
-template <bool F16>
-__device__ __forceinline__ f32x4 mfma16(u32x4 a, u32x4 b, f32x4 c)
-{
-    if constexpr (F16)
-        return __builtin_amdgcn_mfma_f32_16x16x32_f16(__builtin_bit_cast(f16x8, a), __builtin_bit_cast(f16x8, b), c, 0, 0, 0);
-    else
-        return __builtin_amdgcn_mfma_f32_16x16x32_bf16(__builtin_bit_cast(bf16x8, a), __builtin_bit_cast(bf16x8, b), c, 0, 0, 0);
-}
-
-__device__ __forceinline__ int halo_swz(int hx) { return hx & 6; }
-
-__device__ __forceinline__ int xcd_remap_s(int bid, int nwg)
-{
-    const int q = nwg >> 3, r = nwg & 7, xcd = bid & 7;
-    return (xcd < r ? xcd * (q + 1) : r * (q + 1) + (xcd - r) * q) + (bid >> 3);
-}
-
-struct SplitConvArgs {
-    const uint4 *x;
-    const uint4 *w;
-    const float *bias;
-    void *out;
-    int B, H, W, Cin, Cout, cout_pad;
-    float out_scale;
-    int act, out_f32;
-    unsigned *sched;
-    unsigned *status;
-    const float *img;
-    const uint4 *w1;
-    const float *b1;
-    float scale1;
-    long long slab_floats;
-    int ktree;
-};
-
-template <int TH, int WN, int BBUF, int NW, bool F16, bool POOL, bool B1 = false>
+template <int TH, int WN, int BBUF, int NW, bool F16, bool POOL>
 __global__ void __launch_bounds__(64 * NW, NW / 2)
 conv3x3_split_kernel(SplitConvArgs a, int tiles_x, int tiles_y, int n_tiles)
 {
@@ -158,12 +57,9 @@
     static_assert(MI * WM == TH && B_PIECES % NT == 0, "tile shape");
     constexpr int STAGE_LD = 64 + kStagePad;
     constexpr int ABUF = HP * 4 + 4;
-    constexpr int PW = TWS + 4;
-    constexpr int PATCH_F = B1 ? (TH + 4) * PW * 3 : 0;
-    static_assert(!B1 || (WN == 1 && POOL && BBUF == 2), "B1: the 64 -> 64 pooled instantiations only");
     constexpr int LDS_PIPE = 2 * ABUF + BBUF * B_PIECES;
     constexpr int LDS_STAGE = (NW * 32 * STAGE_LD * 4 + 15) / 16;
-    constexpr int LDS_UINT4 = (LDS_PIPE > LDS_STAGE ? LDS_PIPE : LDS_STAGE) + (PATCH_F + 3) / 4;
+    constexpr int LDS_UINT4 = LDS_PIPE > LDS_STAGE ? LDS_PIPE : LDS_STAGE;
 
     __shared__ uint4 lds[LDS_UINT4];
     u32x4 *As = reinterpret_cast<u32x4 *>(lds);
@@ -194,7 +90,7 @@
     const int chunks = a.Cin >> 4;
     const int steps = chunks * 3;
     const size_t in_pix_stride = (size_t)chunks * 4;
-    const uint4 *__restrict__ xin = B1 ? nullptr : a.x + (size_t)img * a.H * a.W * in_pix_stride;
+    const uint4 *__restrict__ xin = a.x + (size_t)img * a.H * a.W * in_pix_stride;
 
     constexpr int A_SLOTS = 3 * A_RPS;
     constexpr unsigned kOob = 0x80000000u;
@@ -203,7 +99,7 @@
     unsigned a_goff[A_SLOTS];
     int a_loff[A_SLOTS];
 #pragma unroll
-    for (int R = 0; R < (B1 ? 0 : A_SLOTS); ++R) {
+    for (int R = 0; R < A_SLOTS; ++R) {
         const int e = R * NT + tid;
         const int pix = e >> 2, pc = e & 3;
         const int hy = pix / HW, hx = pix - hy * HW;
@@ -236,57 +132,6 @@
 #define RPN_LOAD_A(CHUNK, R) \
     __builtin_bit_cast(u32x4, __builtin_amdgcn_raw_buffer_load_b128(xrsrc, a_goff[R], (CHUNK) * 64, 0))
 
-    constexpr int NBLK = (HP + 15) / 16;
-    constexpr int QB = B1 ? (NBLK + NW - 1) / NW : 1;
-    constexpr int QPS = (QB + 2) / 3;
-    float *patchf = reinterpret_cast<float *>(lds + (LDS_PIPE > LDS_STAGE ? LDS_PIPE : LDS_STAGE));
-    const int lr = lane & 15, kg = lane >> 4;
-    u32x4 phi[QB], plo[QB];
-    int pdst[QB];
-    float b1_max = 0.0f;
-    unsigned pin = 0;
-    u32x4 w1hi = {0, 0, 0, 0}, w1lo = {0, 0, 0, 0};
-    f32x4 b1v = {0.f, 0.f, 0.f, 0.f};
-    (void)patchf; (void)lr; (void)kg; (void)pin; (void)phi; (void)plo; (void)pdst; (void)w1hi; (void)w1lo; (void)b1v;
-    (void)b1_max;
-#define RPN_B1_LOADW(CHUNK)                                                                            \
-    {                                                                                                  \
-        const u32x4 *w1_ = reinterpret_cast<const u32x4 *>(a.w1) + ((CHUNK) * 16 + lr) * 8 + kg;       \
-        w1hi = w1_[0];                                                                                 \
-        w1lo = w1_[4];                                                                                 \
-        b1v = *reinterpret_cast<const f32x4 *>(a.b1 + (CHUNK) * 16 + 4 * kg);                          \
-    }
-#define RPN_B1_BLOCK(Q, BUF)                                                                           \
-    {                                                                                                  \
-        f32x4 c_ = {0.f, 0.f, 0.f, 0.f};                                                               \
-        c_ = mfma16<F16>(w1lo, phi[Q], c_);                                                            \
-        c_ = mfma16<F16>(w1hi, plo[Q], c_);                                                            \
-        c_ = mfma16<F16>(w1hi, phi[Q], c_);                                                            \
-        using E_ = typename Half<F16>::elem;                                                           \
-        using h4_ = __attribute__((ext_vector_type(4))) E_;                                            \
-        const bool in_ = (pin >> (Q)) & 1u;                                                            \
-        h4_ hv_, lv_;                                                                                  \
-        _Pragma("unroll") for (int r_ = 0; r_ < 4; ++r_) {                                             \
-            float v_ = fmaxf(c_[r_] * a.scale1 + b1v[r_], 0.0f);                                       \
-            v_ = in_ ? v_ : 0.0f;                                                                      \
-            b1_max = fmaxf(b1_max, v_);                                                                \
-            const E_ h_ = (E_)v_;                                                                      \
-            hv_[r_] = h_;                                                                              \
-            lv_[r_] = (E_)(v_ - (float)h_);                                                            \
-        }                                                                                              \
-        char *d_ = reinterpret_cast<char *>(As + (BUF) * ABUF);                                        \
-        *reinterpret_cast<uint2 *>(d_ + pdst[Q]) = __builtin_bit_cast(uint2, hv_);                     \
-        *reinterpret_cast<uint2 *>(d_ + (pdst[Q] ^ 16)) = __builtin_bit_cast(uint2, lv_);              \
-    }
-    if constexpr (B1) {
-        const float *ximg = a.img + (size_t)img * a.H * a.W * 3;
-        for (int e = tid; e < PATCH_F; e += NT) {
-            const int pr = e / (PW * 3), rem = e - pr * (PW * 3);
-            const int iy = oy0 - 2 + pr, ix = ox0 - 2 + rem / 3;
-            patchf[e] = (iy >= 0 && iy < a.H && ix >= 0 && ix < a.W) ? ximg[((size_t)iy * a.W + ix) * 3 + rem % 3] : 0.0f;
-        }
-    }
-
     f32x16 acc[MI][NI];
 #pragma unroll
     for (int i = 0; i < MI; ++i)
@@ -305,41 +150,10 @@
         b_off[j] = n * 4 + ((2 * kh) ^ ((n >> 2) & 3));
     }
 
-    if constexpr (B1) {
-        RPN_LOAD_B(0);
-        RPN_B1_LOADW(0);
-        RPN_STORE_B(0);
-        __syncthreads();
-        int koff[8];
-#pragma unroll
-        for (int j = 0; j < 8; ++j) {
-            const int k = 8 * kg + j;
-            koff[j] = k < 27 ? (k / 9) * (PW * 3) + (k % 9) : -1;
-        }
-#pragma unroll
-        for (int q = 0; q < QB; ++q) {
-            const int p = (wave + NW * q) * 16 + lr;
-            const bool valid = p < HP;
-            const int pp = valid ? p : HP - 1;
-            const int hy = pp / HW, hx = pp - hy * HW;
-            const int base = (hy * PW + hx) * 3;
-            float xs[8];
-#pragma unroll
-            for (int j = 0; j < 8; ++j) xs[j] = koff[j] >= 0 ? patchf[base + koff[j]] : 0.0f;
-            phi[q] = __builtin_bit_cast(u32x4, split_piece<F16>(xs, false));
-            plo[q] = __builtin_bit_cast(u32x4, split_piece<F16>(xs, true));
-            const int iy = oy0 - 1 + hy, ix = ox0 - 1 + hx;
-            if (iy >= 0 && iy < a.H && ix >= 0 && ix < a.W) pin |= 1u << q;
-            pdst[q] = valid ? (pp * 4 + ((2 * (kg >> 1)) ^ ((hx >> 2) & 3))) * 16 + (kg & 1) * 8 : HP * 4 * 16 + (kg & 1) * 8;
-        }
-#pragma unroll
-        for (int q = 0; q < QB; ++q) RPN_B1_BLOCK(q, 0);
-    } else {
-#pragma unroll
-        for (int R = 0; R < A_SLOTS; ++R) As[a_loff[R]] = RPN_LOAD_A(0, R);
-        RPN_LOAD_B(0);
-        RPN_STORE_B(0);
-    }
+#pragma unroll
+    for (int R = 0; R < A_SLOTS; ++R) As[a_loff[R]] = RPN_LOAD_A(0, R);
+    RPN_LOAD_B(0);
+    RPN_STORE_B(0);
     __syncthreads();
 
     int abuf = 0, bbuf = 0;
@@ -350,12 +164,8 @@
         for (int row = 0; row < 3; ++row) {
             const int step = chunk * 3 + row;
             RPN_LOAD_B(step + 1 < steps ? step + 1 : step);
-            if constexpr (B1) {
-                if (row == 0) RPN_B1_LOADW(next_chunk);
-            } else {
-#pragma unroll
-                for (int q = 0; q < A_RPS; ++q) a_reg[q] = RPN_LOAD_A(next_chunk, row * A_RPS + q);
-            }
+#pragma unroll
+            for (int q = 0; q < A_RPS; ++q) a_reg[q] = RPN_LOAD_A(next_chunk, row * A_RPS + q);
             if constexpr (NW == 4) RPN_PIN_LOADS();
 
             const u32x4 *arow = As + (abuf * ABUF + (wm * MI + row) * HW * 4);
@@ -384,13 +194,8 @@
 
             if (BBUF == 1) __syncthreads();
             RPN_STORE_B(BBUF == 2 ? (bbuf ^ 1) : 0);
-            if constexpr (B1) {
-#pragma unroll
-                for (int q = row * QPS; q < (row + 1) * QPS && q < QB; ++q) RPN_B1_BLOCK(q, abuf ^ 1);
-            } else {
-#pragma unroll
-                for (int q = 0; q < A_RPS; ++q) As[(abuf ^ 1) * ABUF + a_loff[row * A_RPS + q]] = a_reg[q];
-            }
+#pragma unroll
+            for (int q = 0; q < A_RPS; ++q) As[(abuf ^ 1) * ABUF + a_loff[row * A_RPS + q]] = a_reg[q];
             __syncthreads();
             if (BBUF == 2) bbuf ^= 1;
         }
@@ -400,11 +205,6 @@
 #undef RPN_LOAD_B
 #undef RPN_STORE_B
 #undef RPN_LOAD_A
-#undef RPN_B1_LOADW
-#undef RPN_B1_BLOCK
-    if constexpr (B1 && F16) {
-        if (a.status && !(b1_max <= 65504.0f)) atomicOr(a.status, 1u );
-    }
     float *stage = reinterpret_cast<float *>(lds) + wave * (32 * STAGE_LD);
     float bias_v[NI];
 #pragma unroll
@@ -497,118 +297,6 @@
 #else
 #define RPN_STORE_INDEX(i) (i)
 #endif
-
-template <bool F16, bool POOL, int RW, int NW, int NJ = 4>
-__device__ __forceinline__ void split16_epilogue(f32x4 (&acc)[RW * 2][NJ], float *lds_f, const SplitConvArgs &a, int img,
-                                                 int oy0, int ox0, int n0, int wave, int wm, int wn, int lane,
-                                                 int stamp_base = -1 )
-{
-    (void)stamp_base;
-    asm volatile("" : "+v"(lane));
-    constexpr int MT = RW * 2;
-    constexpr int CW = 16 * NJ;
-    constexpr int STAGE_LD = CW + kStagePad;
-    constexpr int PP = CW / 4;
-    const int lr = lane & 15, kg = lane >> 4;
-    float *stage = lds_f + wave * (32 * STAGE_LD);
-    float bias_v[NJ];
-#pragma unroll
-    for (int j = 0; j < NJ; ++j) {
-        const int n = n0 + wn * CW + j * 16 + lr;
-        bias_v[j] = (a.bias && n < a.Cout) ? a.bias[n] : 0.0f;
-    }
-    const float act_lo = a.act == ACT_LINEAR ? -INFINITY : 0.0f;
-    const float act_hi = a.act == ACT_RELU6 ? 6.0f : INFINITY;
-    const int cout_chunks = a.Cout >> 4;
-    const int nbase = n0 + wn * CW;
-    const int pix_bytes = a.out_f32 ? a.Cout * 4 : cout_chunks * 64;
-    constexpr int PXR = 64 / PP;
-    const int px_l = lane / PP, q_l = lane % PP;
-    auto store_stage = [&](int npx_log2, int oy, int oxb, int OHo, int OWo) {
-        if (oy >= OHo) return;
-        const int rounds = (PP << npx_log2) >> 6;
-        const long long row_off = (((long long)img * OHo + oy) * OWo + oxb) * (long long)pix_bytes;
-        const __amdgpu_buffer_rsrc_t ors = __builtin_amdgcn_make_buffer_rsrc(reinterpret_cast<char *>(a.out) + row_off, (short)0,
-                                                                              (OWo - oxb) * pix_bytes, 0x00020000);
-        if (a.out_f32) {
-            const int n = nbase + 4 * q_l;
-            unsigned voff = n < a.Cout ? (unsigned)(px_l * pix_bytes + n * 4) : 0x80000000u;
-#pragma unroll
-            for (int rd = 0; rd < rounds; ++rd) {
-                const u32x4 v = *reinterpret_cast<const u32x4 *>(&stage[(rd * PXR + px_l) * STAGE_LD + 4 * q_l]);
-#ifdef RPN_NOSTORE
-                __builtin_amdgcn_raw_buffer_store_b128(v, ors, (unsigned)(lane * 16), 0, 0);
-#else
-                __builtin_amdgcn_raw_buffer_store_b128(v, ors, voff, 0, 0);
-#endif
-                voff += (unsigned)(PXR * pix_bytes);
-            }
-        } else {
-            constexpr int LPP = CW / 8;
-            constexpr int PXR2 = 64 / LPP;
-            const int px2 = lane / LPP, q2 = lane % LPP;
-            const int cl = q2 >> 1, hf = q2 & 1;
-            const int n = nbase + cl * 16;
-            unsigned voff = n < a.Cout ? (unsigned)(px2 * pix_bytes + (n >> 4) * 64 + hf * 32) : 0x80000000u;
-            const int rounds2 = (1 << npx_log2) / PXR2;
-#pragma unroll
-            for (int rd = 0; rd < rounds2; ++rd) {
-                float xs[8];
-                const float *src = &stage[(rd * PXR2 + px2) * STAGE_LD + cl * 16 + hf * 8];
-                const float4 v0 = *reinterpret_cast<const float4 *>(src);
-                const float4 v1 = *reinterpret_cast<const float4 *>(src + 4);
-                xs[0] = v0.x; xs[1] = v0.y; xs[2] = v0.z; xs[3] = v0.w;
-                xs[4] = v1.x; xs[5] = v1.y; xs[6] = v1.z; xs[7] = v1.w;
-                const u32x4 hi = __builtin_bit_cast(u32x4, split_piece<F16>(xs, false, a.status));
-                const u32x4 lo = __builtin_bit_cast(u32x4, split_piece<F16>(xs, true, nullptr));
-#ifdef RPN_NOSTORE
-                __builtin_amdgcn_raw_buffer_store_b128(hi, ors, (unsigned)(lane * 32), 0, 0);
-                __builtin_amdgcn_raw_buffer_store_b128(lo, ors, (unsigned)(lane * 32 + 16), 0, 0);
-#else
-                __builtin_amdgcn_raw_buffer_store_b128(hi, ors, voff, 0, 0);
-                __builtin_amdgcn_raw_buffer_store_b128(lo, ors, voff + 16u, 0, 0);
-#endif
-                voff += (unsigned)(PXR2 * pix_bytes);
-            }
-        }
-    };
-
-    if constexpr (POOL) {
-        const int OHo = a.H >> 1, OWo = a.W >> 1;
-#pragma unroll
-        for (int hf = 0; hf < 2; ++hf)
-#pragma unroll
-            for (int j = 0; j < NJ; ++j)
-#pragma unroll
-                for (int r2 = 0; r2 < 2; ++r2) {
-                    const float v0 = fmaxf(acc[hf][j][2 * r2], acc[hf][j][2 * r2 + 1]);
-                    const float v1 = fmaxf(acc[(MT - 2) + hf][j][2 * r2], acc[(MT - 2) + hf][j][2 * r2 + 1]);
-                    const int px2 = 8 * hf + 2 * kg + r2;
-                    stage[px2 * STAGE_LD + j * 16 + lr] = fminf(fmaxf(fmaxf(v0, v1) * a.out_scale + bias_v[j], act_lo), act_hi);
-                }
-        wave_sync();
-        store_stage(4, (oy0 + 2 * wm) >> 1, ox0 >> 1, OHo, OWo);
-    } else {
-#pragma unroll
-        for (int i = 0; i < RW; ++i) {
-#pragma unroll
-            for (int hf = 0; hf < 2; ++hf)
-#pragma unroll
-                for (int j = 0; j < NJ; ++j)
-#pragma unroll
-                    for (int r = 0; r < 4; ++r) {
-                        const int px = 16 * hf + 4 * kg + r;
-                        stage[px * STAGE_LD + j * 16 + lr] =
-                            fminf(fmaxf(acc[i * 2 + hf][j][r] * a.out_scale + bias_v[j], act_lo), act_hi);
-                    }
-            wave_sync();
-            if (stamp_base >= 0) RPN_STAMP_AT(stamp_base + 2 * i);
-            store_stage(5, oy0 + RW * wm + i, ox0, a.H, a.W);
-            wave_sync();
-            if (stamp_base >= 0) RPN_STAMP_AT(stamp_base + 2 * i + 1);
-        }
-    }
-}
 
 template <int TH, int WN, int NW, bool F16, bool POOL>
 __global__ void __launch_bounds__(64 * NW, NW == 8 ? 2 : 2)
@@ -2517,27 +2205,4 @@
     return f16 ? launch_split_tiles<true, false>(a, s) : launch_split_tiles<false, false>(a, s);
 }
 
-hipError_t launch_vgg_block1(const float *img, const void *w1, const float *b1, float scale1, const void *w2,
-                             const float *b2, float scale2, void *out, int B, int H, int W, bool f16, hipStream_t s)
-{
-    if (B < 1 || H < 2 || W < 2) return hipErrorInvalidValue;
-    SplitConvArgs a{};
-    a.status = range_status();
-    a.x = nullptr; a.w = (const uint4 *)w2; a.bias = b2; a.out = out;
-    a.B = B; a.H = H; a.W = W; a.Cin = 64; a.Cout = 64; a.cout_pad = 64;
-    a.out_scale = scale2; a.act = ACT_RELU; a.out_f32 = 0;
-    a.img = img; a.w1 = (const uint4 *)w1; a.b1 = b1; a.scale1 = scale1;
-    const int tiles_x = (W + TWS - 1) / TWS, tiles_y = (H + 7) / 8;
-    const long long m_tiles = (long long)tiles_x * tiles_y * B;
-    const long long nblocks = 8ll * ((m_tiles + 7) / 8);
-    if (nblocks > 0x7fffffffll) return hipErrorInvalidValue;
-    if (f16)
-        hipLaunchKernelGGL((conv3x3_split_kernel<8, 1, 2, 4, true, true, true>), dim3((unsigned)nblocks), dim3(256), 0, s, a,
-                           tiles_x, tiles_y, 1);
-    else
-        hipLaunchKernelGGL((conv3x3_split_kernel<8, 1, 2, 4, false, true, true>), dim3((unsigned)nblocks), dim3(256), 0, s, a,
-                           tiles_x, tiles_y, 1);
-    return hipGetLastError();
-}
-
-}
+}
```

Result: no change. 3068 images/s, median of 6 (+0.6%).
